# wenzhang-dev/bitcaskDB

Measured on AMD Instinct MI355X. Metric: WAL record decode+CRC GiB/s (device-resident), 4 KiB values, 1/2/4/8 MI355X, higher is better.
Workload: dtype u8; 1 GPU; config B: 1073743514 B WAL segment per GPU, NsSize 20, 100 B keys, 4 KiB values, device-resident decode+CRC+record parse; seg_bytes=1073743514, records=253846, fragments=286402, parallelism=one independent segment per GPU x1

## Files before the change

### bitcaskdb_amd/csrc/bcw_api.cpp

```cpp
#include <hip/hip_runtime.h>
#include <nmmintrin.h>

#include <algorithm>
#include <atomic>
#include <cmath>
#include <cstdlib>
#include <cstring>
#include <new>
#include <thread>
#include <vector>

#include "bcw.h"
#include "bcw_internal.h"

namespace bcw {

static void byte_table(uint32_t* t0) {
  for (uint32_t b = 0; b < 256; ++b) {
    uint32_t c = b;
    for (int k = 0; k < 8; ++k) c = (c >> 1) ^ (0x82F63B78u & (0u - (c & 1u)));
    t0[b] = c;
  }
}

static inline uint32_t zero_step(const uint32_t* t0, uint32_t s) { return (s >> 8) ^ t0[s & 0xffu]; }

static void shift_basis(const uint32_t* t0, uint64_t n, uint32_t* img) {
  for (int i = 0; i < 32; ++i) {
    uint32_t v = 1u << i;
    for (uint64_t k = 0; k < n; ++k) v = zero_step(t0, v);
    img[i] = v;
  }
}
static inline uint32_t apply_basis(const uint32_t* img, uint32_t x) {
  uint32_t r = 0;
  for (int i = 0; x; ++i, x >>= 1)
    if (x & 1u) r ^= img[i];
  return r;
}

static void invert_basis(const uint32_t* img, uint32_t* inv) {
  uint32_t out[32], in[32];
  for (int i = 0; i < 32; ++i) { out[i] = img[i]; in[i] = 1u << i; }
  for (int bit = 0; bit < 32; ++bit) {
    int p = bit;
    while (p < 32 && !((out[p] >> bit) & 1u)) ++p;
    std::swap(out[bit], out[p]);
    std::swap(in[bit], in[p]);
    for (int r = 0; r < 32; ++r)
      if (r != bit && ((out[r] >> bit) & 1u)) { out[r] ^= out[bit]; in[r] ^= in[bit]; }
  }
  for (int bit = 0; bit < 32; ++bit) inv[bit] = in[bit];
}

static void nibble_image(const uint32_t* img, uint32_t* t) {
  for (int i = 0; i < 8; ++i)
    for (uint32_t n = 0; n < 16; ++n) t[i * 16 + n] = apply_basis(img, n << (4 * i));
}

static void build_enc_ops(uint32_t* ops) {
  uint32_t t0[256];
  byte_table(t0);
  uint32_t img[32], inv[32], sq[32];
  for (int n = 0; n < 16; ++n) { shift_basis(t0, 16ull * n, img); nibble_image(img, ops + n * 128); }
  for (int n = 0; n < 16; ++n) { shift_basis(t0, 256ull * n, img); nibble_image(img, ops + (16 + n) * 128); }
  for (int n = 0; n < 8; ++n) { shift_basis(t0, 4096ull * n, img); nibble_image(img, ops + (32 + n) * 128); }
  for (int t = 0; t < 16; ++t) {
    shift_basis(t0, (uint64_t)t, img);
    invert_basis(img, inv);
    nibble_image(inv, ops + (kOpInv + t) * 128);
  }
  shift_basis(t0, 1, img);
  for (int k = 0; k < 32; ++k) {
    nibble_image(img, ops + (kOpPow2 + k) * 128);
    if (k < 15) {
      invert_basis(img, inv);
      nibble_image(inv, ops + (kOpPow2Inv + k) * 128);
    }
    for (int i = 0; i < 32; ++i) sq[i] = apply_basis(img, img[i]);
    memcpy(img, sq, sizeof img);
  }
}

void build_initc(uint32_t* initc) {
  uint32_t t0[256];
  byte_table(t0);
  uint32_t v = 0xffffffffu;
  for (uint32_t L = 0; L <= kBlock; ++L) {
    initc[L] = v;
    v = zero_step(t0, v);
  }
}

static uint32_t crc32c_hw(const uint8_t* p, size_t n) {
  uint64_t c = 0xffffffffu;
  while (n >= 8) {
    uint64_t w;
    memcpy(&w, p, 8);
    c = _mm_crc32_u64(c, w);
    p += 8;
    n -= 8;
  }
  uint32_t c32 = (uint32_t)c;
  while (n--) c32 = _mm_crc32_u8(c32, *p++);
  return ~c32;
}
static inline uint32_t mask_crc(uint32_t c) { return ((c >> 15) | (c << 17)) + 0xa282ead8u; }

}

using namespace bcw;


#define HIPCHK(x)                          \
  do {                                     \
    if ((x) != hipSuccess) return BCW_E_HIP; \
  } while (0)

namespace {
std::atomic<uint64_t> g_ctx_ids{1};
}

extern "C" {

int bcw_abi_version(void) { return BCW_ABI_VERSION; }

const char* bcw_strerror(int code) {
  switch (code) {
    case BCW_OK: return "ok";
    case BCW_E_INVAL: return "invalid argument";
    case BCW_E_HIP: return "HIP runtime error";
    case BCW_E_NOMEM: return "out of memory";
    case BCW_E_CAPACITY: return "output capacity too small";
    case BCW_E_NODEVICE: return "no HIP device";
    case BCW_E_IO: return "file read / write failed";
    default: return "unknown error";
  }
}

int bcw_device_count(void) {
  int n = 0;
  if (hipGetDeviceCount(&n) != hipSuccess) return 0;
  return n;
}

uint32_t bcw_crc32c_masked(const uint8_t* p, uint64_t n) { return mask_crc(crc32c_hw(p, (size_t)n)); }

void bcw_write_super_block(uint8_t out[40], uint64_t create_time, uint64_t base_time) {
  memset(out, 0, 40);
  const uint64_t magic = BCW_MAGIC, bs = BCW_BLOCK_SIZE;
  const uint32_t so = BCW_SUPER_BLOCK_SIZE;
  memcpy(out + 0, &magic, 8);
  memcpy(out + 8, &bs, 8);
  memcpy(out + 16, &so, 4);
  memcpy(out + 20, &create_time, 8);
  memcpy(out + 28, &base_time, 8);
  const uint32_t crc = bcw_crc32c_masked(out, 36);
  memcpy(out + 36, &crc, 4);
}

int bcw_load_super_block(const uint8_t* p, uint64_t n, bcw_super_block* out) {
  if (!p || !out) return BCW_E_INVAL;
  if (n < BCW_SUPER_BLOCK_SIZE) return BCW_SB_SHORT;
  uint32_t want;
  memcpy(&want, p + 36, 4);
  const uint32_t crc = bcw_crc32c_masked(p, 36);
  if (crc != want) return BCW_SB_CRC;
  memcpy(&out->magic, p, 8);
  if (out->magic != BCW_MAGIC) return BCW_SB_MAGIC;
  memcpy(&out->block_size, p + 8, 8);
  memcpy(&out->start_off, p + 16, 4);
  if (out->block_size != BCW_BLOCK_SIZE) return BCW_SB_BLOCKSIZE;
  memcpy(&out->create_time, p + 20, 8);
  memcpy(&out->base_time, p + 28, 8);
  out->crc = crc;
  return BCW_SB_OK;
}

uint64_t bcw_wal_record_size(uint64_t offset, uint64_t size) {
  uint64_t left = size, phy = 0;
  offset -= BCW_SUPER_BLOCK_SIZE;
  while (left > 0) {
    uint64_t leftover = BCW_BLOCK_SIZE - (offset % BCW_BLOCK_SIZE);
    if (leftover < BCW_HEADER_SIZE) {
      phy += leftover;
      offset += leftover;
      leftover = BCW_BLOCK_SIZE;
    }
    const uint64_t frag = std::min(left, leftover - BCW_HEADER_SIZE);
    phy += BCW_HEADER_SIZE + frag;
    offset += BCW_HEADER_SIZE + frag;
    left -= frag;
  }
  return phy;
}

void bcw_wal_block_index_range(uint64_t offset, uint64_t size, uint64_t* first_blk_idx, uint64_t* first_blk_off,
                               uint64_t* blk_num) {
  const uint64_t rs = bcw_wal_record_size(offset, size);
  const uint64_t first = (offset - BCW_SUPER_BLOCK_SIZE) / BCW_BLOCK_SIZE;
  const uint64_t last = (offset - BCW_SUPER_BLOCK_SIZE + rs) / BCW_BLOCK_SIZE;
  if (first_blk_idx) *first_blk_idx = first;
  if (first_blk_off) *first_blk_off = first * BCW_BLOCK_SIZE + BCW_SUPER_BLOCK_SIZE;
  if (blk_num) *blk_num = last - first + 1;
}

uint64_t bcw_max_fragments(uint64_t seg_len, uint32_t start_off) {
  if (seg_len <= start_off) return 0;
  return (seg_len - start_off) / BCW_HEADER_SIZE + 1;
}

int bcw_ctx_create(int device, bcw_ctx** out) {
  if (!out) return BCW_E_INVAL;
  *out = nullptr;
  int n = 0;
  if (hipGetDeviceCount(&n) != hipSuccess || n == 0) return BCW_E_NODEVICE;
  if (device < 0 || device >= n) return BCW_E_INVAL;
  bcw_ctx* c = new (std::nothrow) bcw_ctx();
  if (!c) return BCW_E_NOMEM;
  c->device = device;
  c->id = g_ctx_ids.fetch_add(1);
  DeviceGuard dg(device);
  if (!dg.ok) { delete c; return BCW_E_HIP; }
  hipDeviceProp_t prop;
  if (hipGetDeviceProperties(&prop, device) == hipSuccess && prop.multiProcessorCount > 0)
    c->num_cus = prop.multiProcessorCount;
  if (hipStreamCreateWithFlags(&c->own, hipStreamNonBlocking) != hipSuccess) { delete c; return BCW_E_HIP; }
  c->cur = c->own;
  std::vector<uint32_t> initc(kBlock + 1);
  build_initc(initc.data());
  std::vector<uint32_t> enc_ops(kEncOpsWords);
  build_enc_ops(enc_ops.data());
  std::vector<uint32_t> pow2(kPow2Ops * 128);
  {
    uint32_t t0[256], img[32], sq[32];
    byte_table(t0);
    shift_basis(t0, 1, img);
    for (int k = 0; k < kPow2Ops; ++k) {
      nibble_image(img, pow2.data() + k * 128);
      for (int i = 0; i < 32; ++i) sq[i] = apply_basis(img, img[i]);
      memcpy(img, sq, sizeof img);
    }
  }
  std::vector<uint32_t> image2(kS2Image);
  {
    uint32_t tk[4][256], t0[256], img[32], nib[128], step[32], m[32];
    byte_table(t0);
    memcpy(tk[0], t0, sizeof t0);
    for (int k = 1; k < 4; ++k)
      for (int e = 0; e < 256; ++e) tk[k][e] = (tk[k - 1][e] >> 8) ^ t0[tk[k - 1][e] & 0xffu];
    uint32_t sh[32];
    shift_basis(t0, kSChunk - kSPiece, sh);
    for (int e = 0; e < 256; ++e)
      for (int s = 0; s < 4; ++s)
        for (int cp = 0; cp < 8; ++cp) {
          image2[kS2SliceOff + e * 64 + s * 8 + cp] = tk[3 - s][e];
          image2[kS2SliceOff + e * 64 + 32 + s * 8 + cp] = apply_basis(sh, tk[3 - s][e]);
        }
    shift_basis(t0, kSPiece, step);
    for (int i = 0; i < 32; ++i) m[i] = 1u << i;
    for (int l = 63; l >= 0; --l) {
      nibble_image(m, nib);
      for (int k = 0; k < 128; ++k) image2[kS2LopOff + k * 64 + l] = nib[k];
      for (int i = 0; i < 32; ++i) m[i] = apply_basis(step, m[i]);
    }
    for (int k = 0; k < kSPW; ++k) {
      shift_basis(t0, 4u * (kSPW - k) + (kSChunk - kSPiece), img);
      for (int t = 0; t < 4; ++t)
        for (uint32_t e = 0; e < 256; ++e)
          image2[kS2KopOff + (k * 4 + t) * 256 + e] = apply_basis(img, e << (8 * t));
    }
    auto put_bytes = [&](int at, const uint8_t (&b)[16]) {
      for (int w = 0; w < 4; ++w)
        image2[at + w] = b[4 * w] | b[4 * w + 1] << 8 | b[4 * w + 2] << 16 | (uint32_t)b[4 * w + 3] << 24;
    };
    for (int n = 0; n < kS2GeN; ++n) {
      uint8_t b[16];
      for (int q = 0; q < 16; ++q) b[q] = q >= n ? 0xff : 0x00;
      put_bytes(kS2Ge + 4 * n, b);
    }
    for (int m = 0; m < kS2JselN; ++m) {
      uint8_t b[16];
      for (int q = 0; q < 16; ++q) {
        const int p = q - (m - 3);
        b[q] = (m < kS2JselN - 1 && p >= 0 && p < 4) ? (uint8_t)(4 + p) : 0x0c;
      }
      put_bytes(kS2Jsel + 4 * m, b);
    }
    for (int g = 0; g < kS2GapN; ++g) {
      uint8_t b[16];
      for (int q = 0; q < 16; ++q) {
        const int p = q - (g - 6);
        b[q] = g == kS2GapN - 1 ? (uint8_t)(q & 3) : (p >= 0 && p < 4) ? (uint8_t)(4 + p) : (p >= 4 && p < 7) ? 0x0c
                                                                                            : (uint8_t)(q & 3);
      }
      put_bytes(kS2Gap + 4 * g, b);
    }
  }
  bool ok = hipMalloc(&c->tabs.lds_image2, image2.size() * 4) == hipSuccess &&
            hipMemcpy(c->tabs.lds_image2, image2.data(), image2.size() * 4, hipMemcpyHostToDevice) == hipSuccess;
  ok = ok && hipMalloc(&c->tabs.initc, initc.size() * 4) == hipSuccess &&
            hipMalloc(&c->tabs.enc_ops, enc_ops.size() * 4) == hipSuccess &&
            hipMalloc(&c->tabs.pow2, pow2.size() * 4) == hipSuccess &&
            hipMalloc(&c->d_eres, sizeof(bcw_encode_result)) == hipSuccess &&
            hipMalloc(&c->d_result, sizeof(bcw_decode_result)) == hipSuccess &&
            hipMalloc(&c->d_ires, sizeof(bcw_index_result)) == hipSuccess;
  ok = ok && hipMemcpy(c->tabs.initc, initc.data(), initc.size() * 4, hipMemcpyHostToDevice) == hipSuccess &&
       hipMemcpy(c->tabs.enc_ops, enc_ops.data(), enc_ops.size() * 4, hipMemcpyHostToDevice) == hipSuccess &&
       hipMemcpy(c->tabs.pow2, pow2.data(), pow2.size() * 4, hipMemcpyHostToDevice) == hipSuccess;
  if (!ok) { bcw_ctx_destroy(c); return BCW_E_NOMEM; }
  *out = c;
  return BCW_OK;
}

static void free_scratch(Scratch& s) {
  (void)hipFree(s.fbase);
  (void)hipFree(s.rbase);
  (void)hipFree(s.bsum);
  (void)hipFree(s.lb);
  (void)hipFree(s.lbe);
  (void)hipFree(s.frags);
  (void)hipFree(s.srec);
  (void)hipFree(s.fok);
  (void)hipFree(s.wstart);
  (void)hipFree(s.xbal);
  (void)hipFree(s.misc);
  s = Scratch{};
}

static void free_enc_scratch(EncScratch& e) {
  void* ptrs[] = {e.sz,    e.mflag, e.dsrc, e.da,      e.hda,       e.hsz,  e.dpos,
                  e.hpos,  e.tiles, e.ev,   e.evb,     e.recdesc,   e.emisc, e.evt,
                  e.hnl,   e.evw,   e.wl};
  for (void* q : ptrs) (void)hipFree(q);
  hipStream_t aux = e.aux;
  hipEvent_t evs[3] = {e.ev_scan, e.ev_hscan, e.ev_desc};
  e = EncScratch{};
  e.aux = aux;
  e.ev_scan = evs[0];
  e.ev_hscan = evs[1];
  e.ev_desc = evs[2];
}

int bcw_ctx_destroy(bcw_ctx* c) {
  if (!c) return BCW_E_INVAL;
  DeviceGuard dg(c->device);
  if (c->cur) (void)hipStreamSynchronize(c->cur);
  free_scratch(c->s);
  free_enc_scratch(c->es);
  if (c->es.aux) (void)hipStreamSynchronize(c->es.aux);
  if (c->es.ev_scan) (void)hipEventDestroy(c->es.ev_scan);
  if (c->es.ev_hscan) (void)hipEventDestroy(c->es.ev_hscan);
  if (c->es.ev_desc) (void)hipEventDestroy(c->es.ev_desc);
  if (c->es.aux) (void)hipStreamDestroy(c->es.aux);
  (void)hipFree(c->tabs.enc_ops);
  (void)hipFree(c->tabs.pow2);
  (void)hipFree(c->d_keep);
  (void)hipFree(c->d_eout);
  (void)hipFree(c->d_eres);
  (void)hipFree(c->tabs.initc);
  (void)hipFree(c->tabs.lds_image2);
  (void)hipFree(c->d_seg);
  (void)hipFree(c->d_tab_mem);
  (void)hipFree(c->d_result);
  (void)hipFree(c->d_ires);
  for (auto& m : c->prof.marks) { (void)hipEventDestroy(m.a); (void)hipEventDestroy(m.b); }
  for (auto e : c->prof.pool) (void)hipEventDestroy(e);
  if (c->own) (void)hipStreamDestroy(c->own);
  delete c;
  return BCW_OK;
}

int bcw_ctx_set_stream(bcw_ctx* c, void* stream) {
  if (!c) return BCW_E_INVAL;
  c->cur = stream ? (hipStream_t)stream : c->own;
  return BCW_OK;
}
void* bcw_ctx_stream(bcw_ctx* c) { return c ? (void*)c->cur : nullptr; }
int bcw_ctx_device(bcw_ctx* c) { return c ? c->device : -1; }
int bcw_ctx_sync(bcw_ctx* c) {
  if (!c) return BCW_E_INVAL;
  return hipStreamSynchronize(c->cur) == hipSuccess ? BCW_OK : BCW_E_HIP;
}

static int ensure_scratch(bcw_ctx* c, uint64_t nblocks, uint64_t frag_cap) {
  Scratch& s = c->s;
  if (nblocks <= s.nblocks_cap && frag_cap <= s.frag_cap && s.misc) return BCW_OK;
  (void)hipStreamSynchronize(c->cur);
  const uint64_t nb = std::max(nblocks, s.nblocks_cap);
  const uint64_t fc = std::max(frag_cap, s.frag_cap);
  free_scratch(s);
  const uint64_t nwg = std::max<uint64_t>(nb / 64 + 2, (uint64_t)c->num_cus + 2);
  bool ok = hipMalloc(&s.fbase, (nb + 1) * 4) == hipSuccess && hipMalloc(&s.rbase, (nb + 1) * 4) == hipSuccess &&
            hipMalloc(&s.bsum, (nb + 1) * sizeof(uint2)) == hipSuccess && hipMalloc(&s.lb, nwg * 8) == hipSuccess &&
            hipMalloc(&s.lbe, nwg * 8) == hipSuccess && hipMalloc(&s.frags, fc * sizeof(Frag)) == hipSuccess &&
            hipMalloc(&s.srec, (fc + 4) * sizeof(uint4)) == hipSuccess &&
            hipMalloc(&s.fok, fc) == hipSuccess &&
            hipMalloc(&s.wstart, ((size_t)c->num_cus * kCrcWaves + 1) * 4) == hipSuccess &&
            hipMalloc(&s.xbal, sizeof(XBal)) == hipSuccess &&
            hipMalloc(&s.misc, 16 * sizeof(uint64_t)) == hipSuccess;
  if (!ok) { free_scratch(s); return BCW_E_NOMEM; }
  s.nblocks_cap = nb;
  s.frag_cap = fc;
  s.nlb = nwg;
  s.epoch = 1;
  s.chase_direct = c->chase_direct;
  XBal xb{};
  for (uint32_t y = 0; y < 8; ++y) xb.w[y] = 65536u;
  if (hipMemcpyHtoDAsync(s.xbal, &xb, sizeof xb, c->cur) != hipSuccess || hipStreamSynchronize(c->cur) != hipSuccess ||
      hipMemsetAsync(s.lb, 0, nwg * 8, c->cur) != hipSuccess || hipMemsetAsync(s.lbe, 0, nwg * 8, c->cur) != hipSuccess ||
      hipMemsetAsync(s.misc, 0, 16 * sizeof(uint64_t), c->cur) != hipSuccess ||
      hipMemsetAsync(s.misc + 14, 0xff, 2 * sizeof(uint64_t), c->cur) != hipSuccess ||
      hipMemsetAsync(s.misc, 0xff, sizeof(uint64_t), c->cur) != hipSuccess) {
    free_scratch(s);
    return BCW_E_HIP;
  }
  return BCW_OK;
}

int bcw_decode_segment_async(bcw_ctx* c, const uint8_t* d_seg, const bcw_decode_params* p,
                             const bcw_record_table* t, bcw_decode_result* d_result) {
  if (!c || !p || !t || !d_result) return BCW_E_INVAL;
  if (p->mode != BCW_MODE_RECORD && p->mode != BCW_MODE_HINT) return BCW_E_INVAL;
  if (!t->foff || !t->size || !t->expire || !t->key_len || !t->val_len || !t->meta_len || !t->first_frag ||
      !t->emit_frag || !t->hdr_size || !t->flags || !t->etag_off || !t->status)
    return BCW_E_INVAL;
  if (p->mode == BCW_MODE_HINT && (!t->aux0 || !t->aux1)) return BCW_E_INVAL;
  if (p->seg_len > BCW_MAX_SEGMENT) return BCW_E_INVAL;
  DeviceGuard dg(c->device);
  if (!dg.ok) return BCW_E_HIP;
  c->last_start_off = p->start_off;
  const uint64_t gen = (c->id << 32) | (++c->gen_seq & 0xffffffffull);
  c->frag_gen = gen;
  bcw_decode_result r{};
  r.err_frag = ~0ull;
  r.first_bad_record = -1;
  r.generation = gen;
  if ((uint64_t)p->start_off > p->seg_len) {
    r.err_class = BCW_ERR_PANIC;
    HIPCHK(hipMemcpyAsync(d_result, &r, sizeof r, hipMemcpyHostToDevice, c->cur));
    return BCW_OK;
  }
  const uint64_t nblocks = (p->seg_len - p->start_off + kBlock - 1) / kBlock;
  if (nblocks == 0 || !d_seg) {
    if (nblocks != 0) return BCW_E_INVAL;
    HIPCHK(hipMemcpyAsync(d_result, &r, sizeof r, hipMemcpyHostToDevice, c->cur));
    return BCW_OK;
  }
  const uint64_t per = p->mode == BCW_MODE_HINT ? 96 : 256;
  uint64_t want = std::max<uint64_t>(65536, (p->seg_len - p->start_off) / per + nblocks * 2);
  want = std::max(want, c->frag_hint);
  want = std::min(want, bcw_max_fragments(p->seg_len, p->start_off) + 64);
  want = std::min<uint64_t>(want, 0xfffffff0ull);
  int rc = ensure_scratch(c, nblocks, want);
  if (rc != BCW_OK) return rc;
  c->s.test_abort_wg = c->test_abort_wg;
  c->test_abort_wg = 0;
  if (launch_decode(d_seg, *p, *t, d_result, c->tabs, c->s, nblocks, gen, c->cur, c->num_cus, &c->prof) !=
      hipSuccess)
    return BCW_E_HIP;
  return BCW_OK;
}

int bcw_decode_fragments_async(bcw_ctx* c, const bcw_frag_table* d_frags) {
  if (!c || !d_frags) return BCW_E_INVAL;
  if (!c->s.misc) return BCW_OK;
  DeviceGuard dg(c->device);
  if (!dg.ok) return BCW_E_HIP;
  const uint64_t n = std::min(c->s.frag_cap, d_frags->capacity);
  return launch_export_frags(c->s, *d_frags, c->last_start_off, c->cur, n, c->tabs.initc) == hipSuccess ? BCW_OK
                                                                                                  : BCW_E_HIP;
}

static const char* kKernelNames[K_NUM] = {"k_chase", "k_crc", "(retired)", "k_enc_prep", "k_enc_scan", "k_events",
                                          "k_write", "k_hint_layout", "k_events_hint"};

int bcw_ctx_reserve_fragments(bcw_ctx* c, uint64_t n) {
  if (!c || n >= 0xfffffff0ull) return BCW_E_INVAL;
  c->frag_hint = std::max(c->frag_hint, n);
  return BCW_OK;
}

int bcw_ctx_set_option(bcw_ctx* c, int option, uint64_t value) {
  if (!c) return BCW_E_INVAL;
  switch (option) {
    case BCW_OPT_CHASE_DIRECT:
      if (value > BCW_CHASE_DIRECT_MAX) return BCW_E_INVAL;
      c->s.chase_direct = (uint32_t)value;
      c->chase_direct = (uint32_t)value;
      return BCW_OK;
    case BCW_OPT_DECODE_PATH:
    case BCW_OPT_DECODE_CHUNKS:
      return value == 1 ? BCW_OK : BCW_E_INVAL;
    case BCW_OPT_XCD_BALANCE:
      if (value > 1) return BCW_E_INVAL;
      c->s.xbal_on = (uint32_t)value;
      return BCW_OK;
    case BCW_OPT_FILTER_SNAPSHOT:
      if (value > 1) return BCW_E_INVAL;
      c->filter_snapshot = value != 0;
      return BCW_OK;
    case BCW_OPT_TEST_ABORT_WAIT: {
      const char* hooks = getenv("BCW_TEST_HOOKS");
      if (!hooks || strcmp(hooks, "1") != 0 || value > 0xffffffffull) return BCW_E_INVAL;
      c->test_abort_wg = value;
      return BCW_OK;
    }
    default:
      return BCW_E_INVAL;
  }
}

int bcw_ctx_set_profiling(bcw_ctx* c, int mask) {
  if (!c) return BCW_E_INVAL;
  c->prof.mask = (uint32_t)mask;
  return BCW_OK;
}

int bcw_ctx_set_profiling_sample(bcw_ctx* c, int every) {
  if (!c || every < 1) return BCW_E_INVAL;
  c->prof.every = (uint32_t)every;
  for (uint32_t& q : c->prof.seq) q = 0;
  return BCW_OK;
}

int bcw_ctx_kernel_times(bcw_ctx* c, double* total_ms, uint64_t* launches, int n) {
  if (!c || n < 0) return BCW_E_INVAL;
  if (hipStreamSynchronize(c->cur) != hipSuccess) return BCW_E_HIP;
  for (int k = 0; k < n; ++k) { if (total_ms) total_ms[k] = 0; if (launches) launches[k] = 0; }
  for (const auto& m : c->prof.marks) {
    float ms = 0;
    if (m.kid < n && hipEventElapsedTime(&ms, m.a, m.b) == hipSuccess) {
      if (total_ms) total_ms[m.kid] += ms;
      if (launches) launches[m.kid] += 1;
    }
    c->prof.pool.push_back(m.a);
    c->prof.pool.push_back(m.b);
  }
  c->prof.marks.clear();
  return K_NUM;
}

const char* bcw_kernel_name(int kid) { return (kid >= 0 && kid < K_NUM) ? kKernelNames[kid] : nullptr; }

int bcw_decode_fragments(bcw_ctx* c, const bcw_frag_table* h, uint64_t* n_total) {
  if (!c || !h) return BCW_E_INVAL;
  if (n_total) *n_total = 0;
  if (!c->s.misc) return BCW_OK;
  DeviceGuard dg(c->device);
  if (!dg.ok) return BCW_E_HIP;
  uint64_t misc[16];
  HIPCHK(hipMemcpyAsync(misc, c->s.misc, sizeof misc, hipMemcpyDeviceToHost, c->cur));
  HIPCHK(hipStreamSynchronize(c->cur));
  const uint64_t total = std::min(misc[4], c->s.frag_cap);
  if (n_total) *n_total = total;
  const uint64_t n = std::min(total, h->capacity);
  if (n == 0) return BCW_OK;
  void* mem = nullptr;
  if (hipMalloc(&mem, n * 19) != hipSuccess) return BCW_E_NOMEM;
  uint8_t* m = (uint8_t*)mem;
  bcw_frag_table d;
  d.capacity = n;
  d.data_off = (uint64_t*)m; m += n * 8;
  d.len = (uint32_t*)m; m += n * 4;
  d.stored_crc = (uint32_t*)m; m += n * 4;
  d.type = m; m += n;
  d.crc_ok = m;
  bool ok = launch_export_frags(c->s, d, c->last_start_off, c->cur, n, c->tabs.initc) == hipSuccess;
  auto cp = [&](void* dst, const void* src, size_t esz) {
    return !dst || hipMemcpyAsync(dst, src, n * esz, hipMemcpyDeviceToHost, c->cur) == hipSuccess;
  };
  ok = ok && cp(h->data_off, d.data_off, 8) && cp(h->len, d.len, 4) && cp(h->stored_crc, d.stored_crc, 4) &&
       cp(h->type, d.type, 1) && cp(h->crc_ok, d.crc_ok, 1);
  ok = ok && hipStreamSynchronize(c->cur) == hipSuccess;
  (void)hipFree(mem);
  return ok ? BCW_OK : BCW_E_HIP;
}

static int ensure_dev_table(bcw_ctx* c, uint64_t cap, bool hint) {
  if (cap <= c->d_tab_cap && c->d_tab_mem) return BCW_OK;
  (void)hipStreamSynchronize(c->cur);
  (void)hipFree(c->d_tab_mem);
  c->d_tab_mem = nullptr;
  const uint64_t n = std::max<uint64_t>(cap, 1);
  const size_t bytes = n * (8 * 5 + 4 * 5 + 4);
  if (hipMalloc(&c->d_tab_mem, bytes) != hipSuccess) { c->d_tab_cap = 0; return BCW_E_NOMEM; }
  uint8_t* m = (uint8_t*)c->d_tab_mem;
  bcw_record_table& t = c->d_tab;
  t.capacity = n;
  t.foff = (uint64_t*)m; m += n * 8;
  t.size = (uint64_t*)m; m += n * 8;
  t.expire = (uint64_t*)m; m += n * 8;
  t.aux0 = (uint64_t*)m; m += n * 8;
  t.aux1 = (uint64_t*)m; m += n * 8;
  t.key_len = (uint32_t*)m; m += n * 4;
  t.val_len = (uint32_t*)m; m += n * 4;
  t.meta_len = (uint32_t*)m; m += n * 4;
  t.first_frag = (uint32_t*)m; m += n * 4;
  t.emit_frag = (uint32_t*)m; m += n * 4;
  t.hdr_size = m; m += n;
  t.flags = m; m += n;
  t.etag_off = m; m += n;
  t.status = m;
  c->d_tab_cap = n;
  (void)hint;
  return BCW_OK;
}

int bcw_decode_segment(bcw_ctx* c, const uint8_t* h_seg, const bcw_decode_params* p,
                       const bcw_record_table* h, bcw_decode_result* h_result) {
  if (!c || !p || !h || !h_result) return BCW_E_INVAL;
  if (p->seg_len && !h_seg) return BCW_E_INVAL;
  DeviceGuard dg(c->device);
  if (!dg.ok) return BCW_E_HIP;
  if (p->seg_len > c->d_seg_cap) {
    (void)hipStreamSynchronize(c->cur);
    (void)hipFree(c->d_seg);
    c->d_seg = nullptr;
    c->d_seg_cap = 0;
    if (hipMalloc(&c->d_seg, p->seg_len) != hipSuccess) return BCW_E_NOMEM;
    c->d_seg_cap = p->seg_len;
  }
  if (p->seg_len) HIPCHK(hipMemcpyAsync(c->d_seg, h_seg, p->seg_len, hipMemcpyHostToDevice, c->cur));
  int rc = ensure_dev_table(c, h->capacity, p->mode == BCW_MODE_HINT);
  if (rc != BCW_OK) return rc;
  for (int attempt = 0; attempt < 3; ++attempt) {
    rc = bcw_decode_segment_async(c, c->d_seg, p, &c->d_tab, c->d_result);
    if (rc != BCW_OK) return rc;
    HIPCHK(hipMemcpyAsync(h_result, c->d_result, sizeof *h_result, hipMemcpyDeviceToHost, c->cur));
    HIPCHK(hipStreamSynchronize(c->cur));
    if (!h_result->retry_frag_capacity) break;
    if (bcw_ctx_reserve_fragments(c, h_result->retry_frag_capacity + 64) != BCW_OK) return BCW_E_CAPACITY;
  }
  if (h_result->retry_frag_capacity) return BCW_E_NOMEM;
  const uint64_t n = std::min(h_result->n_records, h->capacity);
  const bcw_record_table& d = c->d_tab;
  auto cp = [&](void* dst, const void* src, size_t esz) -> bool {
    if (!dst || n == 0) return true;
    return hipMemcpyAsync(dst, src, n * esz, hipMemcpyDeviceToHost, c->cur) == hipSuccess;
  };
  bool ok = cp(h->foff, d.foff, 8) && cp(h->size, d.size, 8) && cp(h->expire, d.expire, 8) &&
            cp(h->aux0, d.aux0, 8) && cp(h->aux1, d.aux1, 8) && cp(h->key_len, d.key_len, 4) &&
            cp(h->val_len, d.val_len, 4) && cp(h->meta_len, d.meta_len, 4) && cp(h->first_frag, d.first_frag, 4) &&
            cp(h->emit_frag, d.emit_frag, 4) && cp(h->hdr_size, d.hdr_size, 1) && cp(h->flags, d.flags, 1) &&
            cp(h->etag_off, d.etag_off, 1) && cp(h->status, d.status, 1);
  if (!ok) return BCW_E_HIP;
  HIPCHK(hipStreamSynchronize(c->cur));
  return h_result->n_records > h->capacity ? BCW_E_CAPACITY : BCW_OK;
}


static int ensure_enc_scratch(bcw_ctx* c, uint64_t rows) {
  EncScratch& e = c->es;
  if (rows <= e.rows_cap && e.emisc) return BCW_OK;
  (void)hipStreamSynchronize(c->cur);
  const uint64_t r = std::max(std::max(rows, e.rows_cap), (uint64_t)1);
  free_enc_scratch(e);
  const uint64_t ntiles = r / enc_tile_items() + 2;
  const uint64_t nwin = r / enc_ev_win() + 2;
  bool ok = hipMalloc(&e.sz, r * 4) == hipSuccess && hipMalloc(&e.mflag, r) == hipSuccess &&
            hipMalloc(&e.dsrc, r * 4) == hipSuccess && hipMalloc(&e.da, (r + 1) * 8) == hipSuccess &&
            hipMalloc(&e.hda, (r + 1) * 8) == hipSuccess && hipMalloc(&e.hsz, r * 4) == hipSuccess &&
            hipMalloc(&e.dpos, r * 8) == hipSuccess && hipMalloc(&e.hpos, r * 8) == hipSuccess &&
            hipMalloc(&e.tiles, ntiles * enc_sizeof_tile()) == hipSuccess &&
            hipMalloc(&e.ev, (r + 2) * enc_sizeof_ev()) == hipSuccess && hipMalloc(&e.evb, nwin * 4) == hipSuccess &&
            hipMalloc(&e.evt, nwin * 32768 * 8) == hipSuccess && hipMalloc(&e.hnl, r * 2) == hipSuccess &&
            hipMalloc(&e.evw, nwin * 12) == hipSuccess &&
            hipMalloc(&e.recdesc, r * enc_sizeof_recdesc()) == hipSuccess && hipMalloc(&e.wl, r * 4) == hipSuccess &&
            hipMalloc(&e.emisc, 64 * sizeof(uint64_t)) == hipSuccess;
  if (!ok) { free_enc_scratch(e); return BCW_E_NOMEM; }
  if (!e.aux && (hipStreamCreateWithFlags(&e.aux, hipStreamNonBlocking) != hipSuccess ||
                 hipEventCreateWithFlags(&e.ev_scan, hipEventDisableTiming) != hipSuccess ||
                 hipEventCreateWithFlags(&e.ev_hscan, hipEventDisableTiming) != hipSuccess ||
                 hipEventCreateWithFlags(&e.ev_desc, hipEventDisableTiming) != hipSuccess))
    return BCW_E_HIP;
  (void)hipMemsetAsync(e.mflag, 0, r, c->cur);
  e.rows_cap = r;
  return BCW_OK;
}

int bcw_encode_segment_async(bcw_ctx* c, const uint8_t* d_src, const bcw_encode_params* p,
                             const bcw_record_table* t, const bcw_decode_result* d_src_result, const uint8_t* d_keep,
                             const bcw_encode_out* o, bcw_encode_result* d_result) {
  if (!c || !p || !t || !d_src_result || !o || !d_result) return BCW_E_INVAL;
  if (p->mode != BCW_ENC_COMPACT && p->mode != BCW_ENC_HINT) return BCW_E_INVAL;
  if (p->hint_pos < BCW_SUPER_BLOCK_SIZE || !o->hint) return BCW_E_INVAL;
  if (p->mode == BCW_ENC_COMPACT && (p->wal_pos < BCW_SUPER_BLOCK_SIZE || !o->wal || !d_keep)) return BCW_E_INVAL;
  if (!t->foff || !t->size || !t->expire || !t->key_len || !t->val_len || !t->meta_len || !t->first_frag ||
      !t->emit_frag || !t->hdr_size || !t->flags || !t->etag_off || !t->status)
    return BCW_E_INVAL;
  if (!c->s.frags) return BCW_E_INVAL;
  if (t->capacity >= 0xffffff00ull) return BCW_E_INVAL;
  DeviceGuard dg(c->device);
  if (!dg.ok) return BCW_E_HIP;
  int rc = ensure_enc_scratch(c, t->capacity);
  if (rc != BCW_OK) return rc;
  EncLaunch L{};
  L.d_src = d_src;
  L.p = *p;
  L.table = *t;
  L.rows = t->capacity;
  L.d_src_result = d_src_result;
  L.d_keep = d_keep;
  L.out = *o;
  L.d_result = d_result;
  L.frags = c->s.frags;
  L.crc_ops = c->tabs.enc_ops;
  L.initc = c->tabs.initc;
  L.num_cus = c->num_cus;
  L.gen = c->frag_gen;
  return launch_encode(L, c->es, c->cur, &c->prof) == hipSuccess ? BCW_OK : BCW_E_HIP;
}

}

namespace bcw {
int sync_decode(bcw_ctx* c, const uint8_t* h_src, const bcw_decode_params& dp, bcw_decode_result& dres) {
  uint64_t cap = std::max<uint64_t>(16, dp.seg_len / 64 + 16);
  if (dp.seg_len > c->d_seg_cap) {
    (void)hipStreamSynchronize(c->cur);
    (void)hipFree(c->d_seg);
    c->d_seg = nullptr;
    c->d_seg_cap = 0;
    if (hipMalloc(&c->d_seg, dp.seg_len) != hipSuccess) return BCW_E_NOMEM;
    c->d_seg_cap = dp.seg_len;
  }
  if (dp.seg_len) HIPCHK(hipMemcpyAsync(c->d_seg, h_src, dp.seg_len, hipMemcpyHostToDevice, c->cur));
  for (;;) {
    int rc = ensure_dev_table(c, cap, dp.mode == BCW_MODE_HINT);
    if (rc != BCW_OK) return rc;
    for (int attempt = 0; attempt < 3; ++attempt) {
      rc = bcw_decode_segment_async(c, c->d_seg, &dp, &c->d_tab, c->d_result);
      if (rc != BCW_OK) return rc;
      HIPCHK(hipMemcpyAsync(&dres, c->d_result, sizeof dres, hipMemcpyDeviceToHost, c->cur));
      HIPCHK(hipStreamSynchronize(c->cur));
      if (!dres.retry_frag_capacity) break;
      if (bcw_ctx_reserve_fragments(c, dres.retry_frag_capacity + 64) != BCW_OK) return BCW_E_CAPACITY;
    }
    if (dres.retry_frag_capacity) return BCW_E_NOMEM;
    if (dres.n_records <= c->d_tab.capacity) return BCW_OK;
    cap = dres.n_records + 16;
  }
}

int ensure_keep(bcw_ctx* c, uint64_t rows) {
  if (rows <= c->d_keep_cap && c->d_keep) return BCW_OK;
  (void)hipStreamSynchronize(c->cur);
  (void)hipFree(c->d_keep);
  c->d_keep = nullptr;
  c->d_keep_cap = 0;
  if (hipMalloc(&c->d_keep, std::max<uint64_t>(rows, 1)) != hipSuccess) return BCW_E_NOMEM;
  c->d_keep_cap = std::max<uint64_t>(rows, 1);
  return BCW_OK;
}

bcw_decode_params src_params(const uint8_t* h_src, const bcw_encode_params* p) {
  bcw_super_block sb{};
  bcw_decode_params dp{};
  dp.seg_len = p->src_len;
  dp.start_off = p->src_start_off;
  dp.ns_size = p->ns_size;
  dp.etag_size = p->etag_size;
  dp.mode = BCW_MODE_RECORD;
  dp.base_time = (bcw_load_super_block(h_src, p->src_len, &sb) == BCW_SB_OK) ? sb.base_time : 0;
  return dp;
}

int encode_run(bcw_ctx* c, const bcw_encode_params* p, const bcw_encode_out* h, bcw_encode_result* h_result,
               bcw_encode_out* d_out) {
  const uint64_t rows = c->d_tab.capacity;
  const uint64_t need = h->wal_cap + h->hint_cap + rows * 8;
  if (need > c->d_eout_cap) {
    (void)hipStreamSynchronize(c->cur);
    (void)hipFree(c->d_eout);
    c->d_eout = nullptr;
    c->d_eout_cap = 0;
    if (hipMalloc(&c->d_eout, need + 64) != hipSuccess) return BCW_E_NOMEM;
    c->d_eout_cap = need;
  }
  uint8_t* m = (uint8_t*)c->d_eout;
  bcw_encode_out& d = *d_out;
  d = bcw_encode_out{};
  d.rec_off = (uint64_t*)m;
  d.rec_off_cap = rows;
  m += rows * 8;
  d.wal = m;
  d.wal_cap = h->wal_cap;
  m += (h->wal_cap + 15) & ~15ull;
  d.hint = (uint8_t*)(((uintptr_t)m + 15) & ~(uintptr_t)15);
  d.hint_cap = h->hint_cap;
  if (p->mode == BCW_ENC_HINT && !d.wal) d.wal = d.hint;
  int rc = bcw_encode_segment_async(c, c->d_seg, p, &c->d_tab, c->d_result, c->d_keep, &d, c->d_eres);
  if (rc != BCW_OK) return rc;
  HIPCHK(hipMemcpyAsync(h_result, c->d_eres, sizeof *h_result, hipMemcpyDeviceToHost, c->cur));
  HIPCHK(hipStreamSynchronize(c->cur));
  if (!h_result->fits) return BCW_E_CAPACITY;
  if (h->rec_off && h->rec_off_cap < h_result->n_in) return BCW_E_CAPACITY;
  return BCW_OK;
}

int encode_copy_out(bcw_ctx* c, const bcw_encode_params* p, const bcw_encode_out* h, const bcw_encode_result& r,
                    const bcw_encode_out& d, const bcw_decode_result& dres) {
  if (h->wal && r.wal_need && p->mode == BCW_ENC_COMPACT)
    HIPCHK(hipMemcpyAsync(h->wal, d.wal, r.wal_need, hipMemcpyDeviceToHost, c->cur));
  if (h->hint && r.hint_need) HIPCHK(hipMemcpyAsync(h->hint, d.hint, r.hint_need, hipMemcpyDeviceToHost, c->cur));
  const uint64_t nr = std::min(r.n_in, d.rec_off_cap);
  if (h->rec_off && nr) HIPCHK(hipMemcpyAsync(h->rec_off, d.rec_off, nr * 8, hipMemcpyDeviceToHost, c->cur));
  HIPCHK(hipStreamSynchronize(c->cur));
  if (h->rec_off)
    for (uint64_t i = nr; i < h->rec_off_cap && i < dres.n_records; ++i) h->rec_off[i] = ~0ull;
  return BCW_OK;
}

int encode_to_host(bcw_ctx* c, const bcw_encode_params* p, const bcw_encode_out* h, bcw_encode_result* h_result,
                   const bcw_decode_result& dres) {
  bcw_encode_out d{};
  const int rc = encode_run(c, p, h, h_result, &d);
  return rc != BCW_OK ? rc : encode_copy_out(c, p, h, *h_result, d, dres);
}
}

extern "C" {

int bcw_encode_segment(bcw_ctx* c, const uint8_t* h_src, const bcw_encode_params* p, const uint8_t* h_keep,
                       uint64_t n_keep, const bcw_encode_out* h, bcw_encode_result* h_result) {
  if (!c || !p || !h || !h_result) return BCW_E_INVAL;
  if (p->src_len && !h_src) return BCW_E_INVAL;
  DeviceGuard dg(c->device);
  if (!dg.ok) return BCW_E_HIP;
  const bcw_decode_params dp = src_params(h_src, p);
  bcw_decode_result dres{};
  int rc = sync_decode(c, h_src, dp, dres);
  if (rc != BCW_OK) return rc;
  const uint64_t rows = c->d_tab.capacity;
  rc = ensure_keep(c, rows);
  if (rc != BCW_OK) return rc;
  HIPCHK(hipMemsetAsync(c->d_keep, 0, rows, c->cur));
  const uint64_t nk = std::min(n_keep, rows);
  if (h_keep && nk) HIPCHK(hipMemcpyAsync(c->d_keep, h_keep, nk, hipMemcpyHostToDevice, c->cur));
  return encode_to_host(c, p, h, h_result, dres);
}

int bcw_compact_segment(bcw_ctx* c, bcw_index* ix, const uint8_t* h_src, const bcw_encode_params* p, uint64_t src_fid,
                        const bcw_encode_out* h, bcw_encode_result* h_result, bcw_index_result* h_filter) {
  if (!c || !ix || !p || !h || !h_result || p->mode != BCW_ENC_COMPACT) return BCW_E_INVAL;
  if (index_ctx(ix) != c) return BCW_E_INVAL;
  if (p->src_len && !h_src) return BCW_E_INVAL;
  DeviceGuard dg(c->device);
  if (!dg.ok) return BCW_E_HIP;
  const bcw_decode_params dp = src_params(h_src, p);
  bcw_decode_result dres{};
  int rc = sync_decode(c, h_src, dp, dres);
  if (rc != BCW_OK) return rc;
  rc = ensure_keep(c, c->d_tab.capacity);
  if (rc != BCW_OK) return rc;
  rc = bcw_compact_filter_async(ix, c->d_seg, &dp, &c->d_tab, c->d_result, src_fid, c->d_keep,
                                h_filter ? c->d_ires : nullptr);
  if (rc != BCW_OK) return rc;
  if (h_filter) HIPCHK(hipMemcpyAsync(h_filter, c->d_ires, sizeof *h_filter, hipMemcpyDeviceToHost, c->cur));
  return encode_to_host(c, p, h, h_result, dres);
}

int bcw_index_recover_segment(bcw_ctx* c, bcw_index* ix, const uint8_t* h_seg, const bcw_decode_params* p,
                              uint64_t fid, int use_record_fid, bcw_decode_result* h_dres,
                              bcw_index_result* h_out) {
  if (!c || !ix || !p || !h_out) return BCW_E_INVAL;
  if (index_ctx(ix) != c) return BCW_E_INVAL;
  if (p->seg_len && !h_seg) return BCW_E_INVAL;
  DeviceGuard dg(c->device);
  if (!dg.ok) return BCW_E_HIP;
  bcw_decode_result dres{};
  int rc = sync_decode(c, h_seg, *p, dres);
  if (rc != BCW_OK) return rc;
  if (h_dres) *h_dres = dres;
  rc = bcw_index_put_decoded_async(ix, c->d_seg, p, &c->d_tab, c->d_result, fid, use_record_fid, c->d_ires);
  if (rc != BCW_OK) return rc;
  HIPCHK(hipMemcpyAsync(h_out, c->d_ires, sizeof *h_out, hipMemcpyDeviceToHost, c->cur));
  HIPCHK(hipStreamSynchronize(c->cur));
  return BCW_OK;
}

namespace {
struct Writer {
  uint8_t* out;
  uint64_t cap;
  uint64_t len;
  void put(const void* p, uint64_t n) {
    if (out && len + n <= cap) memcpy(out + len, p, n);
    len += n;
  }
  uint64_t write_record(const uint8_t* rec, uint64_t n, bool compute_crc) {
    static const uint8_t pad[6] = {0, 0, 0, 0, 0, 0};
    uint64_t offset = 0, left = n;
    bool begin = true;
    while (left > 0) {
      uint64_t leftover = BCW_BLOCK_SIZE - ((len - BCW_SUPER_BLOCK_SIZE) % BCW_BLOCK_SIZE);
      if (leftover < BCW_HEADER_SIZE) {
        put(pad, leftover);
        leftover = BCW_BLOCK_SIZE;
      }
      if (begin) offset = len;
      const uint64_t avail = leftover - BCW_HEADER_SIZE;
      const uint64_t frag = std::min(left, avail);
      const bool end = left == frag;
      const uint8_t type = (begin && end) ? BCW_RECORD_FULL : begin ? BCW_RECORD_FIRST : end ? BCW_RECORD_LAST
                                                                                          : BCW_RECORD_MIDDLE;
      uint8_t hdr[7];
      const uint32_t crc = compute_crc ? mask_crc(crc32c_hw(rec, frag)) : 0;
      const uint16_t l16 = (uint16_t)frag;
      memcpy(hdr, &crc, 4);
      memcpy(hdr + 4, &l16, 2);
      hdr[6] = type;
      put(hdr, 7);
      put(rec, frag);
      rec += frag;
      left -= frag;
      begin = false;
    }
    return offset;
  }
};

inline uint64_t splitmix64(uint64_t& s) {
  uint64_t z = (s += 0x9E3779B97F4A7C15ull);
  z = (z ^ (z >> 30)) * 0xBF58476D1CE4E5B9ull;
  z = (z ^ (z >> 27)) * 0x94D049BB133111EBull;
  return z ^ (z >> 31);
}
inline void fill_rand(uint64_t& s, uint8_t* p, size_t n) {
  size_t i = 0;
  for (; i + 8 <= n; i += 8) {
    const uint64_t v = splitmix64(s);
    memcpy(p + i, &v, 8);
  }
  if (i < n) {
    const uint64_t v = splitmix64(s);
    memcpy(p + i, &v, n - i);
  }
}
inline int put_uvarint(uint8_t* o, uint64_t v) {
  int i = 0;
  while (v >= 0x80) { o[i++] = (uint8_t)(v | 0x80); v >>= 7; }
  o[i++] = (uint8_t)v;
  return i;
}
}

int bcw_synth_segment(uint64_t target_bytes, uint64_t max_records, uint64_t seed, uint32_t ns_size,
                      uint32_t key_len, uint32_t value_len, int value_mode, uint64_t base_time, uint8_t* h_out,
                      uint64_t out_cap, uint64_t* out_len, uint64_t* out_records) {
  if (value_mode != 0 && value_mode != 1) return BCW_E_INVAL;
  if (ns_size > 255 || key_len > (1u << 20) || value_len > (1u << 26)) return BCW_E_INVAL;
  Writer w0{h_out, out_cap, 0};
  uint8_t sb[40];
  bcw_write_super_block(sb, base_time, base_time);
  w0.put(sb, 40);
  std::vector<double> cdf;
  if (value_mode == 1) {
    cdf.resize(512);
    double acc = 0;
    for (int k = 1; k <= 512; ++k) { acc += std::pow((double)k, -1.1); cdf[k - 1] = acc; }
    for (auto& x : cdf) x /= acc;
  }
  const size_t vmax = value_mode == 1 ? 128 * 512 : value_len;
  std::vector<uint8_t> ns(ns_size);
  for (uint32_t i = 0; i < ns_size; ++i) ns[i] = (uint8_t)('A' + i % 26);
  struct Bufs {
    std::vector<uint8_t> key, val, rec;
  };
  auto one = [&](uint64_t i, uint64_t& s, Writer& w, bool fill, Bufs& B) {
    size_t vl = value_len;
    if (value_mode == 1) {
      const double u = (double)(splitmix64(s) >> 11) * (1.0 / 9007199254740992.0);
      vl = 128u * (size_t)(std::lower_bound(cdf.begin(), cdf.end(), u) - cdf.begin() + 1);
    }
    if (fill) {
      fill_rand(s, B.key.data(), key_len);
      if (key_len >= 8) memcpy(B.key.data(), &i, 8);
      fill_rand(s, B.val.data(), vl);
    } else {
      s += 0x9E3779B97F4A7C15ull * (uint64_t)(((key_len + 7) / 8) + ((vl + 7) / 8));
    }
    uint8_t tmp[30];
    int t = 0;
    t += put_uvarint(tmp + t, key_len);
    t += put_uvarint(tmp + t, vl);
    t += put_uvarint(tmp + t, 0);
    const size_t header = (size_t)t + ns_size + 2;
    const size_t n = header + key_len + vl;
    if (!fill) {
      w.write_record(B.rec.data(), n, false);
      return;
    }
    uint8_t* r = B.rec.data();
    size_t o = 0;
    r[o++] = (uint8_t)header;
    memcpy(r + o, ns.data(), ns_size); o += ns_size;
    r[o++] = (uint8_t)((1u << 0) | (1u << 1));
    memcpy(r + o, tmp, t); o += t;
    memcpy(r + o, B.key.data(), key_len); o += key_len;
    memcpy(r + o, B.val.data(), vl); o += vl;
    w.write_record(r, o, true);
  };
  auto bufs = [&]() {
    Bufs B;
    B.key.resize(key_len + 8);
    B.val.resize(vmax + 8);
    B.rec.resize(vmax + key_len + ns_size + 64);
    return B;
  };
  constexpr uint64_t kCk = 4096;
  struct Ck {
    uint64_t i, s, len;
  };
  std::vector<Ck> ck;
  Writer wl{nullptr, 0, w0.len};
  uint64_t s = seed, n = 0;
  Bufs B0 = bufs();
  for (uint64_t i = 0; (max_records == 0 || i < max_records) && wl.len < target_bytes; ++i) {
    if (i % kCk == 0) ck.push_back(Ck{i, s, wl.len});
    one(i, s, wl, false, B0);
    ++n;
  }
  if (out_len) *out_len = wl.len;
  if (out_records) *out_records = n;
  if (!h_out) return BCW_OK;
  if (wl.len > out_cap) return BCW_E_CAPACITY;
  const unsigned hw = std::thread::hardware_concurrency();
  const uint64_t nth = std::max<uint64_t>(1, std::min<uint64_t>({(uint64_t)(hw ? hw : 1), 16, ck.size()}));
  std::atomic<uint64_t> next{0};
  auto fill = [&]() {
    Bufs B = bufs();
    for (uint64_t c; (c = next.fetch_add(1)) < ck.size();) {
      Writer w{h_out, out_cap, ck[c].len};
      uint64_t st = ck[c].s;
      const uint64_t i1 = std::min<uint64_t>(ck[c].i + kCk, n);
      for (uint64_t i = ck[c].i; i < i1; ++i) one(i, st, w, true, B);
    }
  };
  std::vector<std::thread> pool;
  for (uint64_t t = 1; t < nth; ++t) pool.emplace_back(fill);
  fill();
  for (auto& t : pool) t.join();
  return BCW_OK;
}

}
```

### bitcaskdb_amd/csrc/bcw_decode.hip

```cpp
#include <hip/hip_runtime.h>

#include <cstdint>

#include "bcw_internal.h"
#include "bcw_parse.h"

namespace bcw {

enum { M_FIRST_BAD = 0,
       M_NE = 1,
       M_NFRAGS = 4, M_DONE_CRC = 5,
       M_T_CRC0 = 10, M_T_FIN = 11,
       M_ABORT = 12,
       M_BAD_CRC = 14,
       M_BAD_TYPE = 15 };

__device__ __forceinline__ uint32_t rotl32(uint32_t x, int r) { return (x << r) | (x >> (32 - r)); }

__device__ __forceinline__ void read_header(const uint8_t* __restrict__ seg, uint64_t seg_len, uint64_t off,
                                            uint32_t& crc, uint32_t& len, uint32_t& type) {
  const uint64_t a = off & ~3ull;
  uint32_t w0, w1, w2;
  if (a + 12 <= seg_len) {
    const uint32_t* q = reinterpret_cast<const uint32_t*>(seg + a);
    w0 = q[0]; w1 = q[1]; w2 = q[2];
  } else {
    uint32_t b[12];
#pragma unroll
    for (int i = 0; i < 12; ++i) b[i] = (a + i < seg_len) ? seg[a + i] : 0u;
    w0 = b[0] | b[1] << 8 | b[2] << 16 | b[3] << 24;
    w1 = b[4] | b[5] << 8 | b[6] << 16 | b[7] << 24;
    w2 = b[8] | b[9] << 8 | b[10] << 16 | b[11] << 24;
  }
  const uint32_t sh = (uint32_t)(off & 3);
  crc = __builtin_amdgcn_alignbyte(w1, w0, sh);
  const uint32_t t = __builtin_amdgcn_alignbyte(w2, w1, sh);
  len = t & 0xffffu;
  type = (t >> 16) & 0xffu;
}

__device__ __forceinline__ uint32_t wave_incl_scan_u32(uint32_t v, uint32_t lane) {
#pragma unroll
  for (int d = 1; d < 64; d <<= 1) {
    const uint32_t t = __shfl_up(v, d, 64);
    if (lane >= (uint32_t)d) v += t;
  }
  return v;
}
template <int CTRL>
__device__ __forceinline__ uint32_t dpp_mov(uint32_t v) {
  return (uint32_t)__builtin_amdgcn_mov_dpp((int)v, CTRL, 0xf, 0xf, false);
}
template <int CTRL, int ROWMASK = 0xf>
__device__ __forceinline__ uint32_t dpp_z(uint32_t v) {
  return (uint32_t)__builtin_amdgcn_update_dpp(0, (int)v, CTRL, ROWMASK, 0xf, true);
}
template <typename Op>
__device__ __forceinline__ uint32_t wave_scan_z(uint32_t v, Op op) {
  v = op(v, dpp_z<0x111>(v));
  v = op(v, dpp_z<0x112>(v));
  v = op(v, dpp_z<0x114>(v));
  v = op(v, dpp_z<0x118>(v));
  v = op(v, dpp_z<0x142, 0xa>(v));
  v = op(v, dpp_z<0x143, 0xc>(v));
  return v;
}
__device__ __forceinline__ uint32_t wave_max_scan(uint32_t v, uint32_t) {
  return wave_scan_z(v, [](uint32_t x, uint32_t y) { return max(x, y); });
}
__device__ __forceinline__ uint32_t wave_or_scan(uint32_t v, uint32_t) {
  return wave_scan_z(v, [](uint32_t x, uint32_t y) { return x | y; });
}
__device__ __forceinline__ uint32_t wave_add_scan(uint32_t v, uint32_t) {
  return wave_scan_z(v, [](uint32_t x, uint32_t y) { return x + y; });
}

__device__ __forceinline__ uint32_t wg256_excl_scan(uint32_t v, uint32_t* sm4, uint32_t& total) {
  const uint32_t lane = threadIdx.x & 63u, wave = threadIdx.x >> 6;
  const uint32_t incl = wave_incl_scan_u32(v, lane);
  if (lane == 63) sm4[wave] = incl;
  __syncthreads();
  uint32_t base = 0;
  for (uint32_t k = 0; k < wave; ++k) base += sm4[k];
  total = sm4[0] + sm4[1] + sm4[2] + sm4[3];
  __syncthreads();
  return base + incl - v;
}

struct Spin {
  uint64_t t0 = 0;
  uint64_t lim = 20000000ull;
  __device__ __forceinline__ bool go(uint64_t* misc, uint32_t site) {
    const uint64_t t = wall_clock64();
    if (t0 == 0) t0 = t;
    if (t - t0 < lim &&
        __hip_atomic_load(&misc[M_ABORT], __ATOMIC_RELAXED, __HIP_MEMORY_SCOPE_AGENT) == 0ull) {
      __builtin_amdgcn_s_sleep(1);
      return true;
    }
    atomicMax(reinterpret_cast<unsigned long long*>(&misc[M_ABORT]), (unsigned long long)site);
    return false;
  }
};

constexpr int kChaseHold = 64;
constexpr uint64_t kLbAgg = 1, kLbInc = 2, kLbMask = (1ull << 38) - 1;
constexpr int kDirect = BCW_CHASE_DIRECT_MAX;

template <typename V>
__device__ __forceinline__ uint32_t chase_block(const uint8_t* __restrict__ seg, uint64_t seg_len, uint64_t boff,
                                                uint32_t bufsize, V&& visit, uint32_t h = 0, uint32_t n = 0) {
  while (h + kHdr <= bufsize) {
    uint32_t crc, len, type;
    read_header(seg, seg_len, boff + h, crc, len, type);
    const uint32_t start = h + kHdr;
    if (len > bufsize - start) len = bufsize - start;
    visit(n, start, len, crc, type);
    ++n;
    h = start + len;
  }
  return n;
}

constexpr uint32_t kRecUsual = 1u << 20, kRecAdj = 1u << 21;
__device__ __forceinline__ uint32_t check_word(uint32_t crc, uint32_t ic) { return ~rotl32(crc - 0xa282ead8u, 15) ^ ic; }
__device__ __forceinline__ void put_frag_J(Frag* __restrict__ frags, uint4* __restrict__ srec, uint64_t g,
                                           uint64_t frag_cap, uint32_t b, uint64_t boff, uint32_t start_len,
                                           uint32_t J, uint32_t type, bool adj) {
  if (g >= frag_cap) return;
  *reinterpret_cast<uint4*>(frags + g) = make_uint4(b, start_len, J, type & 0xffu);
  const uint64_t gs = boff + (start_len & 0xffffu), ge = gs + (start_len >> 16);
  const uint32_t cb = (uint32_t)(gs / kSChunk), ce = (uint32_t)(ge / kSChunk);
  const uint32_t pa = (uint32_t)(gs % kSChunk), pb = (uint32_t)(ge % kSChunk);
  const bool usual = adj && cb < ce && pb <= (uint32_t)kSChunk - 8u;
  const uint32_t e = pb + 4u, K = ((e % kSPiece) + 3u) >> 2, Lfull = e / kSPiece + (K == (uint32_t)kSPW ? 1u : 0u);
  srec[g] = make_uint4(ce, cb, J, pb | pa << 10 | (usual ? kRecUsual : 0u) | (adj ? kRecAdj : 0u) | Lfull << 22 |
                                      (K & 3u) << 29);
}
__device__ __forceinline__ void put_frag(Frag* __restrict__ frags, uint4* __restrict__ srec, uint64_t g,
                                         uint64_t frag_cap, uint32_t b, uint64_t boff, uint32_t start, uint32_t len,
                                         uint32_t crc, uint32_t type, const uint32_t* __restrict__ initc, bool adj) {
  put_frag_J(frags, srec, g, frag_cap, b, boff, start | (len << 16), check_word(crc, initc[len]), type, adj);
}

constexpr uint32_t kSumHasE = 1u << 16;

struct ClassW {
  uint64_t pw;
  uint64_t pp0, pp1;
  uint64_t p8;
  __device__ __forceinline__ uint64_t weight(uint32_t y) const {
    return (uint64_t)(65536 + 256 * (int64_t)(int8_t)(uint8_t)(pw >> (8u * y)));
  }
  __device__ __forceinline__ uint64_t prefix(uint32_t y) const {
    const uint64_t f = (y < 4u ? pp0 : pp1) >> (16u * (y & 3u));
    return (uint64_t)(65536 * (int64_t)y + 256 * (int64_t)(int16_t)(uint16_t)f);
  }
  __device__ __forceinline__ uint32_t classes_below(double x) const {
    uint32_t n = 0;
#pragma unroll
    for (uint32_t k = 1; k < 8; ++k) n += (double)prefix(k) <= x ? 1u : 0u;
    return n;
  }
};
__device__ __forceinline__ uint64_t div_floor(uint64_t a, uint64_t b, double rb) {
  uint64_t q = (uint64_t)((double)a * rb);
  while (q * b > a) --q;
  while ((q + 1) * b <= a) ++q;
  return q;
}
struct WavePart {
  ClassW cw;
  uint64_t L, nwaves, round16, den16, C;
  double rden, rC;
  __device__ __forceinline__ WavePart(const ClassW& c, uint64_t L_, uint64_t nwaves_) : cw(c), L(L_), nwaves(nwaves_) {
    const uint32_t G = (uint32_t)(nwaves / kCrcWaves);
    round16 = 16ull * cw.p8;
    den16 = round16 * (G / 8u) + 16ull * cw.prefix(G % 8u);
    C = L / 1024u;
    rden = 1.0 / (double)den16;
    rC = C ? 1.0 / (double)C : 0.0;
  }
  __device__ __forceinline__ uint64_t P(uint64_t v) const {
    if (v >= nwaves) return L;
    const uint64_t r = v / kCrcWaves;
    const uint32_t y = (uint32_t)(r % 8u);
    const uint64_t num16 = round16 * (r / 8u) + 16ull * cw.prefix(y) + cw.weight(y) * (v % kCrcWaves);
    return 1024u * div_floor(num16 * C, den16, rden);
  }
  __device__ __forceinline__ uint64_t first_at(uint64_t x) const {
    if (C == 0) return x == 0 ? 0 : nwaves;
    const uint64_t X = (x + 1023u) / 1024u, N = div_floor(X * den16 + C - 1, C, rC);
    const uint32_t q = (uint32_t)N / (uint32_t)round16;
    const uint64_t rem = N - (uint64_t)q * round16;
    uint32_t y = 0;
#pragma unroll
    for (uint32_t k = 1; k < 8; ++k) y += 16ull * cw.prefix(k) <= rem ? 1u : 0u;
    const uint64_t wy = cw.weight(y), base = 16ull * cw.prefix(y);
    const uint32_t jj = (uint32_t)(rem - base + wy - 1) / (uint32_t)wy;
    const uint64_t v = ((uint64_t)q * 8u + y) * kCrcWaves + jj;
    return v < nwaves ? v : nwaves;
  }
};

__device__ __forceinline__ ClassW class_weights(uint32_t xw) {
  ClassW c{0, 0, 0, 0};
  int64_t acc = 0;
#pragma unroll
  for (int k = 0; k < 8; ++k) {
    const int64_t d = ((int64_t)__builtin_amdgcn_readlane(xw, k) - 65536) / 256;
    c.pw |= (uint64_t)(uint8_t)(int8_t)d << (8 * k);
    if (k < 4) c.pp0 |= (uint64_t)(uint16_t)(int16_t)acc << (16 * k);
    else c.pp1 |= (uint64_t)(uint16_t)(int16_t)acc << (16 * (k - 4));
    acc += d;
  }
  c.p8 = (uint64_t)(65536 * 8 + 256 * acc);
  return c;
}

template <int ABL = 0>
__global__ __launch_bounds__(64) void k_chase(const uint8_t* __restrict__ seg, uint64_t seg_len, uint32_t start_off,
                                              uint64_t nblocks, uint32_t* __restrict__ fbase,
                                              uint32_t* __restrict__ rbase, uint2* __restrict__ bsum,
                                              Frag* __restrict__ frags, uint4* __restrict__ srec, uint64_t frag_cap,
                                              uint64_t* __restrict__ lb,
                                              uint64_t* __restrict__ lbe, uint64_t* __restrict__ misc,
                                              uint64_t epoch, const uint32_t* __restrict__ initc,
                                              uint32_t direct_max, uint64_t test_abort_wg,
                                              uint32_t* __restrict__ wstart, uint32_t nwaves,
                                              XBal* __restrict__ xb, uint32_t xb_on) {
  constexpr int kHold = (ABL & 256) ? 16 : kChaseHold;
  __shared__ uint32_t s_hold[kHold][2][64];
  __shared__ uint8_t s_type[kHold][64];
  const uint32_t lane = threadIdx.x;
  const uint32_t xw = lane < 8u ? (xb_on ? xb->w[lane] : 65536u) : 0u;
  const uint64_t tc0 = (ABL & 16) ? __builtin_amdgcn_s_memtime() : 0;
  if ((ABL & 32) && threadIdx.x == 0) lbe[4 * blockIdx.x] = wall_clock64();
  const uint64_t wg = blockIdx.x;
  if (wg >= (nblocks + 63) / 64) return;
  const uint64_t b = wg * 64 + lane;
  uint32_t bufsize = 0;
  uint64_t boff = 0;
  if (b < nblocks) {
    boff = (uint64_t)start_off + b * kBlock;
    bufsize = (uint32_t)((seg_len - boff) < kBlock ? (seg_len - boff) : kBlock);
  }
  uint32_t ne = 0, tacc = 0, tnz = 0xffffu, tst = 0, badk = 0xffffffffu;
  uint32_t hres = 0;
  const uint32_t n = chase_block(seg, seg_len, boff, bufsize,
                                 [&](uint32_t k, uint32_t start, uint32_t len, uint32_t crc, uint32_t type) {
                                   if (k < (uint32_t)kHold) {
                                     s_hold[k][0][lane] = crc;
                                     s_hold[k][1][lane] = start | (len << 16);
                                     s_type[k][lane] = (uint8_t)type;
                                   }
                                   if (k == (uint32_t)kHold - 1u) hres = start + len;
                                   if (type == BCW_RECORD_FULL || type == BCW_RECORD_LAST) {
                                     ++ne;
                                     tacc = 0;
                                     tnz = 0xffffu;
                                   } else {
                                     if (len > 0 && tnz == 0xffffu) { tnz = k; tst = start; }
                                     tacc += len;
                                     if ((type < BCW_RECORD_FULL || type > BCW_RECORD_LAST) && badk == 0xffffffffu) badk = k;
                                   }
                                 });
  const uint64_t tc1 = (ABL & 16) ? __builtin_amdgcn_s_memtime() : 0;
  if ((ABL & 32) && lane == 0) lbe[4 * wg + 1] = wall_clock64();
  if (wg == 0 && lane == 0) xb->on = xb_on;
  const uint32_t incl = wave_add_scan(n, lane);
  const uint32_t tot = __builtin_amdgcn_readlane(incl, 63);
  const uint32_t incl_e = wave_add_scan(ne, lane);
  const uint32_t tot_e = __builtin_amdgcn_readlane(incl_e, 63);
  const uint64_t tag = epoch << 40;
  const uint64_t nwg_all = (nblocks + 63) / 64;
  const bool force = wg + 1 == test_abort_wg;
  uint64_t excl = 0, excl_e = 0;
  const uint32_t nh = n < (uint32_t)kHold ? n : (uint32_t)kHold;
  auto held_checks = [&]() {
    if (ABL & 2) return;
    constexpr uint32_t kWb = 16;
    static_assert(kHold % kWb == 0, "held-header batches stay inside s_hold");
    for (uint32_t k0 = 0; k0 < nh; k0 += kWb) {
      uint32_t ic[kWb];
#pragma unroll
      for (uint32_t q = 0; q < kWb; ++q) ic[q] = initc[k0 + q < nh ? s_hold[k0 + q][1][lane] >> 16 : 0u];
#pragma unroll
      for (uint32_t q = 0; q < kWb; ++q)
        if (k0 + q < nh) s_hold[k0 + q][0][lane] = check_word(s_hold[k0 + q][0][lane], ic[q]);
    }
  };
  if (ABL & 1) {
    held_checks();
  } else if (nwg_all <= (uint64_t)direct_max) {
    if (lane == 0)
      __hip_atomic_store(&lb[wg], tag | (kLbAgg << 38) | tot | ((uint64_t)tot_e << 19), __ATOMIC_RELAXED,
                         __HIP_MEMORY_SCOPE_AGENT);
    uint64_t v[kDirect / 64];
#pragma unroll
    for (int k = 0; k < kDirect / 64; ++k) {
      const uint64_t q = lane + 64u * k;
      v[k] = q < wg ? __hip_atomic_load(&lb[q], __ATOMIC_RELAXED, __HIP_MEMORY_SCOPE_AGENT) : tag;
    }
    held_checks();
    Spin sp;
    if (force) sp.lim = 0;
    for (;;) {
      bool wait = force;
#pragma unroll
      for (int k = 0; k < kDirect / 64; ++k) wait |= (v[k] >> 40) != epoch;
      if (!__builtin_amdgcn_readfirstlane((uint32_t)(__ballot(wait) != 0ull))) break;
      if (!sp.go(misc, 9)) {
#pragma unroll
        for (int k = 0; k < kDirect / 64; ++k)
          if ((v[k] >> 40) != epoch) v[k] = 0;
        break;
      }
#pragma unroll
      for (int k = 0; k < kDirect / 64; ++k) {
        const uint64_t q = lane + 64u * k;
        if ((v[k] >> 40) != epoch) v[k] = __hip_atomic_load(&lb[q], __ATOMIC_RELAXED, __HIP_MEMORY_SCOPE_AGENT);
      }
    }
    uint64_t c = 0, ce = 0;
#pragma unroll
    for (int k = 0; k < kDirect / 64; ++k) {
      const uint64_t q = lane + 64u * k;
      if (q < wg) {
        c += v[k] & 0x7ffffu;
        ce += (v[k] >> 19) & 0x7ffffu;
      }
    }
#pragma unroll
    for (int d = 32; d >= 1; d >>= 1) {
      c += (uint64_t)__shfl_xor((long long)c, d, 64);
      ce += (uint64_t)__shfl_xor((long long)ce, d, 64);
    }
    excl = c;
    excl_e = ce;
  } else {
    const uint64_t fl = (wg == 0 ? kLbInc : kLbAgg) << 38;
    if (lane == 0) {
      __hip_atomic_store(&lb[wg], tag | fl | tot, __ATOMIC_RELAXED, __HIP_MEMORY_SCOPE_AGENT);
      __hip_atomic_store(&lbe[wg], tag | fl | tot_e, __ATOMIC_RELAXED, __HIP_MEMORY_SCOPE_AGENT);
    }
    held_checks();
    bool dn = false, de = false;
    for (uint64_t top = wg; top > 0 && !(dn && de);) {
      const uint64_t q = top - 1 - lane;
      uint64_t vn = 0, ve = 0;
      if (top > lane) {
        Spin sp;
        if (force) sp.lim = 0;
        if (!dn)
          while (((vn = __hip_atomic_load(&lb[q], __ATOMIC_RELAXED, __HIP_MEMORY_SCOPE_AGENT)) >> 40) != epoch || force)
            if (!sp.go(misc, 10)) { vn = 0; break; }
        if (!de)
          while (((ve = __hip_atomic_load(&lbe[q], __ATOMIC_RELAXED, __HIP_MEMORY_SCOPE_AGENT)) >> 40) != epoch || force)
            if (!sp.go(misc, 11)) { ve = 0; break; }
      }
      auto step = [&](uint64_t v, bool& done, uint64_t& acc) {
        if (done) return;
        const uint64_t inc = __ballot(top > lane && ((v >> 38) & 3u) == kLbInc);
        const uint32_t stop = inc ? (uint32_t)__builtin_ctzll(inc) : 64u;
        uint64_t c = (lane <= stop && top > lane) ? (v & kLbMask) : 0ull;
#pragma unroll
        for (int d = 32; d >= 1; d >>= 1) c += (uint64_t)__shfl_xor((long long)c, d, 64);
        acc += c;
        done = inc != 0;
      };
      step(vn, dn, excl);
      step(ve, de, excl_e);
      top = top > 64 ? top - 64 : 0;
    }
    if (lane == 0 && wg != 0) {
      __hip_atomic_store(&lb[wg], tag | (kLbInc << 38) | ((excl + tot) & kLbMask), __ATOMIC_RELAXED,
                         __HIP_MEMORY_SCOPE_AGENT);
      __hip_atomic_store(&lbe[wg], tag | (kLbInc << 38) | ((excl_e + tot_e) & kLbMask), __ATOMIC_RELAXED,
                         __HIP_MEMORY_SCOPE_AGENT);
    }
  }
  const uint64_t g0 = excl + incl - n;
  const uint64_t tc2 = (ABL & 16) ? __builtin_amdgcn_s_memtime() : 0;
  if ((ABL & 32) && lane == 0) lbe[4 * wg + 2] = wall_clock64();
  if (b < nblocks && !(ABL & 2)) {
    fbase[b] = (uint32_t)(g0 < 0xffffffffull ? g0 : 0xffffffffull);
    const uint64_t r0 = excl_e + incl_e - ne;
    rbase[b] = (uint32_t)(r0 < 0xffffffffull ? r0 : 0xffffffffull);
    bsum[b] = make_uint2(tacc | (tnz << 16), tst | (ne ? kSumHasE : 0u));
    if (badk != 0xffffffffu)
      atomicMin(reinterpret_cast<unsigned long long*>(&misc[M_BAD_TYPE]), (unsigned long long)(g0 + badk));
    const bool next_hdr = b + 1 < nblocks && seg_len - (boff + kBlock) >= kHdr;
    auto adj = [&](uint32_t k, uint32_t sl_k) { return k + 1u < n || (next_hdr && (sl_k & 0xffffu) + (sl_k >> 16) == kBlock); };
    const uint64_t L = seg_len - start_off, rel = boff - start_off;
    const WavePart wp(class_weights(xw), L, nwaves);
    const uint64_t span = b + 1 == nblocks ? ~0ull : (uint64_t)kBlock - 1;
    uint64_t w = wp.first_at(rel);
    uint64_t bw = wp.P(w) - rel;
    auto bounds_upto = [&](uint64_t hp, uint64_t idx) __attribute__((always_inline)) {
      const uint64_t h = hp < span ? hp : span;
      while (w <= nwaves && bw <= h) {
        wstart[w] = (uint32_t)(idx < 0xffffffffull ? idx : 0xffffffffull);
        ++w;
        bw = wp.P(w) - rel;
      }
    };
    for (uint32_t k = 0; k < nh; ++k) {
      const uint32_t sl = s_hold[k][1][lane];
      put_frag_J(frags, srec, g0 + k, frag_cap, (uint32_t)b, boff, sl, s_hold[k][0][lane], s_type[k][lane],
                 adj(k, sl));
      bounds_upto((sl & 0xffffu) - kHdr, g0 + k);
    }
    if (n > (uint32_t)kHold)
      chase_block(seg, seg_len, boff, bufsize, [&](uint32_t k, uint32_t start, uint32_t len, uint32_t crc, uint32_t type) {
        put_frag(frags, srec, g0 + k, frag_cap, (uint32_t)b, boff, start, len, crc, type, initc,
                 adj(k, start | (len << 16)));
        bounds_upto(start - kHdr, g0 + k);
      }, hres, (uint32_t)kHold);
    bounds_upto(~0ull, g0 + n);
  }
  if (ABL & 32) {
    asm volatile("s_waitcnt vmcnt(0)" ::: "memory");
    if (lane == 0) lbe[4 * wg + 3] = wall_clock64();
  }
  if (ABL & 16) {
    asm volatile("s_waitcnt vmcnt(0)" ::: "memory");
    const uint64_t tc3 = __builtin_amdgcn_s_memtime();
    if (lane == 0) {
      atomicAdd(reinterpret_cast<unsigned long long*>(&misc[7]), (unsigned long long)(tc1 - tc0));
      atomicAdd(reinterpret_cast<unsigned long long*>(&misc[8]), (unsigned long long)(tc2 - tc1));
      atomicAdd(reinterpret_cast<unsigned long long*>(&misc[9]), (unsigned long long)(tc3 - tc2));
    }
  }
  const uint64_t nwg = (nblocks + 63) / 64;
  if (lane == 63 && !(ABL & 2)) {
    const uint64_t total = excl + tot, total_e = excl_e + tot_e;
    const uint64_t be = wg * 64 + 64 < nblocks ? wg * 64 + 64 : nblocks;
    fbase[be] = (uint32_t)(total < 0xffffffffull ? total : 0xffffffffull);
    rbase[be] = (uint32_t)(total_e < 0xffffffffull ? total_e : 0xffffffffull);
    if (wg == nwg - 1) {
      misc[M_NFRAGS] = total;
      misc[M_NE] = total_e;
    }
  }
}

__device__ __forceinline__ uint32_t xor3(uint32_t a, uint32_t b, uint32_t c) {
  return __builtin_amdgcn_bitop3_b32(a, b, c, 0x96);
}
__device__ __forceinline__ uint32_t apply_fwd(const uint32_t* __restrict__ fwd, uint32_t lane, uint32_t x) {
  const uint8_t* b = reinterpret_cast<const uint8_t*>(fwd);
  const uint32_t lane4 = 4u * lane;
  auto at = [&](int i) -> uint32_t {
    const uint32_t sh = 4 * i >= 8 ? (x >> (4 * i - 8)) : (x << (8 - 4 * i));
    return *reinterpret_cast<const uint32_t*>(b + (((sh & 0xf00u) | lane4) + 4096u * (uint32_t)i));
  };
  const uint32_t r0 = at(0), r1 = at(1), r2 = at(2), r3 = at(3), r4 = at(4), r5 = at(5), r6 = at(6), r7 = at(7);
  return xor3(xor3(r0, r1, r2), xor3(r3, r4, r5), r6) ^ r7;
}
__device__ __forceinline__ uint32_t apply_op(const uint32_t* __restrict__ c, uint32_t x) {
  uint32_t r = 0;
#pragma unroll
  for (int i = 0; i < 8; ++i) r ^= c[i * 16 + ((x >> (4 * i)) & 15u)];
  return r;
}

__device__ __forceinline__ uint4 load16_slow(const uint8_t* __restrict__ seg, uint64_t seg_len, int64_t o) {
  uint64_t lo = 0, hi = 0;
#pragma unroll 1
  for (int i = 0; i < 16; ++i) {
    const int64_t q = o + i;
    const uint64_t byte = (q >= 0 && (uint64_t)q < seg_len) ? seg[q] : 0u;
    if (i < 8) lo |= byte << (8 * i); else hi |= byte << (8 * (i - 8));
  }
  return make_uint4((uint32_t)lo, (uint32_t)(lo >> 32), (uint32_t)hi, (uint32_t)(hi >> 32));
}
__device__ __forceinline__ uint4 load16_safe(const uint8_t* __restrict__ seg, uint64_t seg_len, int64_t o) {
  if (o >= 0 && (uint64_t)o + 16 <= seg_len) return *reinterpret_cast<const uint4*>(seg + o);
  return load16_slow(seg, seg_len, o);
}


template <int N>
__device__ __forceinline__ uint32_t reg_byte(const uint32_t (&h)[N], uint32_t pos) {
  uint32_t t[N];
#pragma unroll
  for (int i = 0; i < N; ++i) t[i] = h[i];
  const uint32_t wi = pos >> 2;
  int n = N;
#pragma unroll
  for (int bit = 0; bit < 6; ++bit) {
    if (n <= 1) break;
    const bool hi = (wi >> bit) & 1u;
#pragma unroll
    for (int i = 0; i < (N + 1) / 2; ++i) {
      if (i < (n + 1) / 2) t[i] = (2 * i + 1 < n) ? (hi ? t[2 * i + 1] : t[2 * i]) : t[2 * i];
    }
    n = (n + 1) / 2;
  }
  return (t[0] >> (8u * (pos & 3u))) & 0xffu;
}

constexpr int kHeadWords = 16;
constexpr int kTailWords = 8;

__device__ __attribute__((noinline)) uint32_t walk_byte(const uint8_t* __restrict__ seg, const Frag* __restrict__ frags,
                                                        uint32_t start_off, uint32_t f_first, uint32_t f_last,
                                                        uint64_t pos) {
  uint64_t beg = 0;
  for (uint32_t cf = f_first;; ++cf) {
    const Frag f = frags[cf];
    if (pos < beg + f.len || cf >= f_last)
      return seg[(uint64_t)start_off + (uint64_t)f.blk * kBlock + f.start + (pos - beg)];
    beg += f.len;
  }
}

struct RegReader {
  uint32_t h[kHeadWords];
  uint32_t t[kTailWords];
  uint32_t nhead;
  uint64_t tstart;
  uint64_t tend;
  const uint8_t* seg;
  const Frag* frags;
  uint32_t start_off;
  uint32_t f_first, f_last;
  __device__ __forceinline__ uint32_t operator()(uint64_t pos) {
    if (pos < nhead) return reg_byte(h, (uint32_t)pos);
    if (pos >= tstart && pos < tend) return reg_byte(t, (uint32_t)(pos - tstart));
    return walk_byte(seg, frags, start_off, f_first, f_last, pos);
  }
};

template <int N>
__device__ __forceinline__ void load_words(const uint8_t* __restrict__ seg, uint64_t seg_len, uint64_t base,
                                           uint32_t (&w)[N]) {
  if (base + 4u * N <= seg_len) {
#pragma unroll
    for (int k = 0; k < N / 4; ++k) {
      uint4 v;
      __builtin_memcpy(&v, seg + base + 16 * k, 16);
      w[4 * k + 0] = v.x; w[4 * k + 1] = v.y; w[4 * k + 2] = v.z; w[4 * k + 3] = v.w;
    }
  } else {
#pragma unroll
    for (int k = 0; k < N / 4; ++k) {
      const uint4 v = load16_safe(seg, seg_len, (int64_t)(base + 16 * k));
      w[4 * k + 0] = v.x; w[4 * k + 1] = v.y; w[4 * k + 2] = v.z; w[4 * k + 3] = v.w;
    }
  }
}

struct EmitArgs {
  const uint8_t* seg;
  uint64_t seg_len;
  bcw_decode_params p;
  const Frag* frags;
  const uint32_t* fbase;
  const uint32_t* rbase;
  const uint2* bsum;
  bcw_record_table tab;
  uint64_t* misc;
  uint32_t kb_flags;
  uint64_t* kb_stamps;
};


struct EmitState {
  uint64_t acc;
  int64_t nzb;
  uint32_t nzk, nzs;
  uint64_t rec;
};
__device__ __forceinline__ uint2 emit_prefetch(const EmitArgs& A, uint64_t b0, uint32_t lane) {
  return b0 > lane ? A.bsum[b0 - 1 - lane] : make_uint2(0xffff0000u, kSumHasE);
}

__device__ __forceinline__ EmitState emit_state(const EmitArgs& A, uint64_t b0, uint32_t lane, uint2 s, uint32_t rec) {
  EmitState st{0, -1, 0, 0, rec};
  uint64_t acc = 0;
  for (uint64_t top = b0; top > 0;) {
    if (top != b0) {
      const uint64_t q = top - 1 - lane;
      s = top > lane ? A.bsum[q] : make_uint2(0xffff0000u, kSumHasE);
    }
    const uint64_t he = __ballot((s.y & kSumHasE) != 0u);
    const uint32_t stop = he ? (uint32_t)__builtin_ctzll(he) : 63u;
    const bool contrib = lane <= stop;
    uint32_t ta = contrib ? (s.x & 0xffffu) : 0u;
#pragma unroll
    for (int d = 32; d >= 1; d >>= 1) ta += (uint32_t)__shfl_xor((int)ta, d, 64);
    acc += (uint32_t)__builtin_amdgcn_readfirstlane(ta);
    const uint64_t nzm = __ballot(contrib && (s.x >> 16) != 0xffffu);
    if (nzm) {
      const uint32_t L = 63u - __builtin_clzll(nzm);
      st.nzb = (int64_t)(top - 1 - L);
      st.nzk = (uint32_t)__builtin_amdgcn_readlane((int)(s.x >> 16), L);
      st.nzs = (uint32_t)__builtin_amdgcn_readlane((int)(s.y & 0xffffu), L);
    }
    if (he) break;
    top = top > 64 ? top - 64 : 0;
  }
  st.acc = acc;
  return st;
}

template <bool NOSTORE = false, bool NOPARSE = false, typename Hook>
__device__ __forceinline__ void emit_chunks(const EmitArgs& A, const EmitState& es, uint64_t f0, uint64_t f1,
                                            uint32_t lane, Hook&& hook) {
  if (f0 >= f1) {
    hook();
    return;
  }
  const Frag* __restrict__ frags = A.frags;
  const uint32_t start_off = A.p.start_off;
  uint64_t acc = es.acc, off = 0;
  uint32_t first = 0;
  if (es.nzb >= 0) {
    off = (uint64_t)start_off + (uint64_t)es.nzb * kBlock + es.nzs;
    first = A.fbase[es.nzb] + es.nzk;
  }
  uint64_t rec = es.rec;
  const bool hint = A.p.mode == BCW_MODE_HINT;
  for (uint64_t c0 = f0; c0 < f1; c0 += 64) {
    const uint64_t g = c0 + lane;
    const bool valid = g < f1;
    const uint4 fr = reinterpret_cast<const uint4*>(frags)[valid ? g : f1 - 1];
    if (c0 == f0) hook();
    Frag f;
    __builtin_memcpy(&f, &fr, sizeof f);
    if (!valid) f = Frag{};
    const uint32_t len = valid ? f.len : 0u;
    const uint64_t D = (uint64_t)start_off + (uint64_t)f.blk * kBlock + f.start;
    const bool isE = valid && (f.type == BCW_RECORD_FULL || f.type == BCW_RECORD_LAST);
    const uint64_t E = __ballot(isE);
    const uint64_t NZ = __ballot(valid && len > 0);
    const uint32_t S = wave_add_scan(len, lane);
    const uint64_t below = (lane == 0) ? 0ull : (~0ull >> (64 - lane));
    const uint64_t pm = E & below;
    const int prev = pm ? 63 - __builtin_clzll(pm) : -1;
    const uint32_t S_prev = __shfl(S, prev < 0 ? 0 : prev, 64);
    const uint64_t between = (uint64_t)(S - len) - (prev < 0 ? 0u : S_prev);
    const uint64_t acc_before = (prev < 0 ? acc : 0ull) + between;
    const uint64_t range = prev < 0 ? below : (below & ~(~0ull >> (63 - prev)));
    const uint64_t nzr = NZ & range;
    const int fnz = nzr ? __builtin_ctzll(nzr) : 0;
    const uint64_t D_fnz = __shfl(D, fnz, 64);
    const uint64_t V = __ballot(valid);
    const int last_valid = V ? 63 - __builtin_clzll(V) : -1;
    const uint32_t S_tot = __shfl(S, last_valid < 0 ? 0 : last_valid, 64);
    const int lastE = E ? 63 - __builtin_clzll(E) : -1;
    uint64_t acc2, off2;
    uint32_t first2;
    {
      const uint32_t S_lastE = __shfl(S, lastE < 0 ? 0 : lastE, 64);
      const uint64_t after = lastE < 0 ? V : (V & ~(~0ull >> (63 - lastE)));
      const uint64_t nza = NZ & after;
      const int fa = nza ? __builtin_ctzll(nza) : 0;
      const uint64_t D_fa = __shfl(D, fa, 64);
      if (lastE >= 0) {
        acc2 = (uint64_t)(S_tot - S_lastE);
        off2 = D_fa;
        first2 = (uint32_t)(c0 + fa);
      } else {
        acc2 = acc + S_tot;
        if (acc > 0 || !nza) { off2 = off; first2 = first; }
        else { off2 = D_fa; first2 = (uint32_t)(c0 + fa); }
      }
    }
    uint64_t foff;
    uint32_t ffrag;
    if (acc_before == 0) { foff = D; ffrag = (uint32_t)g; }
    else if (prev < 0 && acc > 0) { foff = off; ffrag = first; }
    else { foff = D_fnz; ffrag = (uint32_t)(c0 + fnz); }
    const bool full = f.type == BCW_RECORD_FULL;
    const uint32_t src = full ? (uint32_t)g : ffrag;
    const bool src_here = src >= c0 && src < c0 + 64;
    const uint32_t sw0 = (uint32_t)__shfl((int)f.blk, src_here ? (int)(src - c0) : (int)lane, 64);
    const uint32_t sw1 = (uint32_t)__shfl((int)((uint32_t)f.start | ((uint32_t)f.len << 16)),
                                          src_here ? (int)(src - c0) : (int)lane, 64);
    const bool nx_here = src + 1u >= c0 && src + 1u < c0 + 64;
    const uint32_t sx0 = (uint32_t)__shfl((int)f.blk, nx_here ? (int)(src + 1u - c0) : (int)lane, 64);
    const uint32_t sx1 = (uint32_t)__shfl((int)((uint32_t)f.start | ((uint32_t)f.len << 16)),
                                          nx_here ? (int)(src + 1u - c0) : (int)lane, 64);
    if (isE) {
      const uint64_t size = full ? (uint64_t)len : acc_before + len;
      const uint64_t r = rec + __builtin_popcountll(E & below);
      Frag fs = f;
      if (!full) {
        if (src_here) { fs.blk = sw0; fs.start = (uint16_t)sw1; fs.len = (uint16_t)(sw1 >> 16); }
        else fs = frags[src];
      }
      RegReader rd;
      const uint64_t a0 = (uint64_t)start_off + (uint64_t)fs.blk * kBlock + fs.start;
      uint64_t want = size < 64u ? size : 64u;
      if (want > fs.len) want = fs.len;
      rd.nhead = (uint32_t)want;
      load_words(A.seg, A.seg_len, a0, rd.h);
      rd.tstart = rd.tend = ~0ull;
      if (hint) {
        uint64_t nt = size < 32u ? size : 32u;
        if (nt > len) nt = len;
        rd.tstart = size - nt;
        load_words(A.seg, A.seg_len, D + len - nt, rd.t);
      } else if (want < (size < 64u ? size : 64u)) {
        Frag f2;
        if (nx_here) { f2.blk = sx0; f2.start = (uint16_t)sx1; f2.len = (uint16_t)(sx1 >> 16); }
        else f2 = frags[src + 1u];
        load_words(A.seg, A.seg_len, (uint64_t)start_off + (uint64_t)f2.blk * kBlock + f2.start, rd.t);
        uint64_t n2 = f2.len < 32u ? f2.len : 32u;
        if (n2 > size - want) n2 = size - want;
        rd.tstart = want;
        rd.tend = want + n2;
      } else {
#pragma unroll
        for (int k = 0; k < kTailWords; ++k) rd.t[k] = 0;
      }
      rd.seg = A.seg; rd.frags = frags; rd.start_off = start_off;
      rd.f_first = src; rd.f_last = (uint32_t)g;
      uint8_t status, hdr, flags, etag_off;
      uint64_t key_len, val_len, meta_len, expire, aux0, aux1;
      if (NOPARSE) {
        status = 0; hdr = (uint8_t)rd.h[0]; flags = (uint8_t)rd.h[5]; etag_off = 0;
        key_len = rd.h[6] ^ rd.h[9]; val_len = rd.h[7] ^ rd.h[12]; meta_len = rd.h[8] ^ rd.h[15]; expire = rd.h[10];
        aux0 = rd.t[0]; aux1 = rd.t[1];
      } else {
        parse_record(A.p, rd, size, status, hdr, flags, etag_off, key_len, val_len, meta_len, expire, aux0, aux1);
      }
      const bcw_record_table& tab = A.tab;
      if (NOSTORE) {
        if (status == 0xeeu) tab.foff[r] = foff ^ size ^ expire ^ aux0 ^ aux1 ^ key_len ^ val_len ^ meta_len ^ hdr ^ flags ^ etag_off;
      } else if (r < tab.capacity) {
        tab.foff[r] = foff;
        tab.size[r] = size;
        tab.expire[r] = expire;
        if (tab.aux0) tab.aux0[r] = aux0;
        if (tab.aux1) tab.aux1[r] = aux1;
        tab.key_len[r] = (uint32_t)key_len;
        tab.val_len[r] = (uint32_t)val_len;
        tab.meta_len[r] = (uint32_t)meta_len;
        tab.first_frag[r] = src;
        tab.emit_frag[r] = (uint32_t)g;
        tab.hdr_size[r] = hdr;
        tab.flags[r] = flags;
        tab.etag_off[r] = etag_off;
        tab.status[r] = status;
      }
      if (status != BCW_ST_OK) atomicMin((unsigned long long*)&A.misc[M_FIRST_BAD], (unsigned long long)r);
    }
    rec += __builtin_popcountll(E);
    acc = acc2;
    off = off2;
    first = first2;
  }
}

struct ItemMeta {
  uint64_t bb;
  uint2 s;
  uint32_t f0, f1, rec;
};
__device__ __forceinline__ uint32_t ld_const(const uint32_t* p, uint64_t i) {
  return ((const __attribute__((address_space(4))) uint32_t*)p)[i];
}
__device__ __forceinline__ ItemMeta item_meta(const EmitArgs& A, uint64_t it, uint64_t bpw, uint64_t cb0, uint64_t cb1,
                                              uint32_t lane) {
  ItemMeta m;
  m.bb = cb0 + it * bpw < cb1 ? cb0 + it * bpw : cb1 - 1;
  const uint64_t be = m.bb + bpw < cb1 ? m.bb + bpw : cb1;
  m.s = emit_prefetch(A, m.bb, lane);
  m.f0 = ld_const(A.fbase, m.bb);
  m.f1 = ld_const(A.fbase, be);
  m.rec = ld_const(A.rbase, m.bb);
  return m;
}

__device__ __forceinline__ void finalize(const EmitArgs& A, uint64_t nblocks, uint64_t frag_cap, uint32_t tail_panic, uint64_t gen,
                         bcw_decode_result* __restrict__ res, uint32_t lane) {
  uint64_t* misc = A.misc;
  const uint64_t bad_crc = __hip_atomic_load(&misc[M_BAD_CRC], __ATOMIC_RELAXED, __HIP_MEMORY_SCOPE_AGENT);
  const uint64_t bad_type = __hip_atomic_load(&misc[M_BAD_TYPE], __ATOMIC_RELAXED, __HIP_MEMORY_SCOPE_AGENT);
  const uint64_t fb = __hip_atomic_load(&misc[M_FIRST_BAD], __ATOMIC_RELAXED, __HIP_MEMORY_SCOPE_AGENT);
  const uint64_t nfr = __hip_atomic_load(&misc[M_NFRAGS], __ATOMIC_RELAXED, __HIP_MEMORY_SCOPE_AGENT);
  const uint64_t abort_site = __hip_atomic_load(&misc[M_ABORT], __ATOMIC_RELAXED, __HIP_MEMORY_SCOPE_AGENT);
  const uint64_t err = bad_crc < bad_type ? bad_crc : bad_type;
  uint64_t lim = err < frag_cap ? err : frag_cap;
  uint64_t nrec = __hip_atomic_load(&misc[M_NE], __ATOMIC_RELAXED, __HIP_MEMORY_SCOPE_AGENT);
  if (lim < nfr && abort_site == 0ull) {
    uint64_t lo = 0, hi = nblocks;
    while (hi - lo > 1) {
      const uint64_t step = (hi - lo + 63) / 64;
      const uint64_t q = lo + (uint64_t)lane * step;
      const bool le = q < hi && A.fbase[q] <= lim;
      const uint64_t m = __ballot(le);
      const uint32_t L = m ? 63u - __builtin_clzll(m) : 0u;
      lo = lo + (uint64_t)L * step;
      hi = lo + step < hi ? lo + step : hi;
    }
    uint64_t cnt = 0;
    for (uint64_t c0 = A.fbase[lo]; c0 < lim; c0 += 64) {
      const uint64_t g = c0 + lane;
      const uint32_t ty = g < lim ? A.frags[g].type : 0u;
      cnt += (uint64_t)__builtin_popcountll(__ballot(ty == BCW_RECORD_FULL || ty == BCW_RECORD_LAST));
    }
    nrec = (uint64_t)A.rbase[lo] + cnt;
  }
  if (lane != 0) return;
  bcw_decode_result r{};
  r.n_records = nrec;
  r.n_records_total = nrec;
  r.err_frag = err;
  r.err_class = err == ~0ull ? BCW_ERR_NONE : (bad_crc <= bad_type ? BCW_ERR_CRC : BCW_ERR_TYPE);
  r.n_frags = err != ~0ull ? err + 1 : nfr;
  if (r.err_class == BCW_ERR_NONE && tail_panic) r.err_class = BCW_ERR_PANIC;
  if (abort_site != 0ull) {
    r.err_class = BCW_ERR_INTERNAL;
    r.err_frag = abort_site;
    r.n_records = r.n_records_total = 0;
    nrec = 0;
  }
  r.err_file_off = 0;
  if (err != ~0ull && err < frag_cap && abort_site == 0ull) {
    const Frag f = A.frags[err];
    r.err_file_off = (uint64_t)A.p.start_off + (uint64_t)f.blk * kBlock + f.start - kHdr;
  }
  r.first_bad_record = fb < nrec ? (int32_t)(fb < 0x7fffffffull ? fb : 0x7fffffffull) : -1;
  r.n_blocks = nblocks;
  r.retry_frag_capacity = (nfr > frag_cap && abort_site == 0ull) ? nfr : 0;
  r.generation = gen;
  *res = r;
  if (abort_site != 0ull) misc[M_NFRAGS] = 0;
  misc[M_DONE_CRC] = 0;
  misc[M_BAD_CRC] = ~0ull;
  misc[M_FIRST_BAD] = ~0ull;
  misc[M_BAD_TYPE] = ~0ull;
  misc[M_ABORT] = 0;
}

struct StreamFrag {
  int64_t gs, ge;
  uint32_t J;
};

struct SliceLane2 {
  uint32_t base;
  uint32_t sel[4];
};
__device__ __forceinline__ SliceLane2 slice_lane2(uint32_t lane) {
  SliceLane2 s;
  const uint32_t g = (lane >> 3) & 3u, copy = lane & 7u;
  s.base = 0;
#pragma unroll
  for (uint32_t k = 0; k < 4; ++k) {
    const uint32_t slot = (k + g) & 3u;
    s.base |= (slot * 32u + copy * 4u) << (8u * k);
    s.sel[k] = 0x0c0c0000u | ((4u + slot) << 8) | k;
  }
  return s;
}
template <bool SH>
__device__ __forceinline__ uint32_t slice4_step2(const uint8_t* __restrict__ tb, const SliceLane2& sl, uint32_t x,
                                                 uint32_t next) {
  constexpr uint32_t o = SH ? 128u : 0u;
  const uint32_t a0 = *reinterpret_cast<const uint32_t*>(tb + __builtin_amdgcn_perm(x, sl.base, sl.sel[0]) + o);
  const uint32_t a1 = *reinterpret_cast<const uint32_t*>(tb + __builtin_amdgcn_perm(x, sl.base, sl.sel[1]) + o);
  const uint32_t a2 = *reinterpret_cast<const uint32_t*>(tb + __builtin_amdgcn_perm(x, sl.base, sl.sel[2]) + o);
  const uint32_t a3 = *reinterpret_cast<const uint32_t*>(tb + __builtin_amdgcn_perm(x, sl.base, sl.sel[3]) + o);
  return xor3(xor3(a0, a1, a2), a3, next);
}
template <bool CAP>
__device__ __forceinline__ uint32_t chain_piece2(const uint8_t* __restrict__ tb, const SliceLane2& sl, uint32_t seed,
                                                 const uint32_t (&w)[kSPW], uint32_t K = 0, uint32_t* cap = nullptr) {
  uint32_t x = seed ^ w[0];
  uint32_t st[kSPW - 1];
#pragma unroll
  for (int q = 0; q < kSPW - 1; ++q) {
    x = slice4_step2<false>(tb, sl, x, w[q + 1]);
    if (CAP) st[q] = x ^ w[q + 1];
  }
  if (CAP) *cap = K == 1u ? st[0] : (K == 2u ? st[1] : st[2]);
  return slice4_step2<true>(tb, sl, x, 0u);
}

__device__ __forceinline__ uint64_t c_safe_bound(uint64_t seg_len) { return (seg_len + 4u + kSChunk - 1u) / kSChunk; }

__device__ __forceinline__ uint4 lds_entry(const uint32_t* __restrict__ tab, uint32_t idx) {
  return *reinterpret_cast<const uint4*>(tab + 4u * idx);
}
__device__ __forceinline__ void mask_gap(uint32_t (&x)[kSPW], const uint32_t (&w)[kSPW], int32_t pb, uint32_t J,
                                         uint32_t lane, const uint32_t* __restrict__ lds) {
  const uint32_t g = min((uint32_t)(pb - (int32_t)(kSPiece * lane) + 6), (uint32_t)(kS2GapN - 1));
  const uint4 S = lds_entry(lds + kS2Gap, g);
  x[0] = __builtin_amdgcn_perm(J, w[0], S.x);
  x[1] = __builtin_amdgcn_perm(J, w[1], S.y);
  x[2] = __builtin_amdgcn_perm(J, w[2], S.z);
  x[3] = __builtin_amdgcn_perm(J, w[3], S.w);
}
__device__ __forceinline__ void mask_chunk(uint32_t (&x)[kSPW], const uint32_t (&w)[kSPW], int32_t pa, int32_t pb,
                                           int32_t pc, uint32_t J, uint32_t lane, const uint32_t* __restrict__ lds) {
  const int32_t q = (int32_t)(kSPiece * lane);
  const uint4 A = lds_entry(lds + kS2Ge, (uint32_t)min(max(pa - q, 0), kS2GeN - 1));
  const uint4 B = lds_entry(lds + kS2Ge, (uint32_t)min(max(pb - q, 0), kS2GeN - 1));
  const uint4 C = lds_entry(lds + kS2Ge, (uint32_t)min(max(pc - q, 0), kS2GeN - 1));
  const uint4 Js = lds_entry(lds + kS2Jsel, min((uint32_t)(pb - q + 3), (uint32_t)(kS2JselN - 1)));
  auto one = [&](uint32_t wj, uint32_t a, uint32_t b, uint32_t c, uint32_t js) {
    const uint32_t keep = __builtin_amdgcn_bitop3_b32(a, b, c, 0xBA);
    const uint32_t sel = __builtin_amdgcn_bitop3_b32(keep, 0x03020100u, js, 0xCA);
    return __builtin_amdgcn_perm(J, wj, sel);
  };
  x[0] = one(w[0], A.x, B.x, C.x, Js.x);
  x[1] = one(w[1], A.y, B.y, C.y, Js.y);
  x[2] = one(w[2], A.z, B.z, C.z, Js.z);
  x[3] = one(w[3], A.w, B.w, C.w, Js.w);
}
__device__ __forceinline__ uint32_t apply_op_b(const uint32_t* __restrict__ t, uint32_t x) {
  const uint32_t a0 = t[x & 0xffu], a1 = t[256 + ((x >> 8) & 0xffu)];
  const uint32_t a2 = t[512 + ((x >> 16) & 0xffu)], a3 = t[768 + (x >> 24)];
  return xor3(a0, a1, a2) ^ a3;
}

template <bool FASTONLY = false>
__device__ __forceinline__ void stream_verify(const uint8_t* __restrict__ seg, uint64_t seg_len,
                                              uint8_t* __restrict__ fok, const uint4* __restrict__ srec, uint64_t f0,
                                              uint32_t nfr, const uint32_t* __restrict__ lds, uint32_t lane,
                                              uint64_t* __restrict__ misc, uint32_t* __restrict__ s_rem,
                                              uint32_t wslot, const uint8_t* __restrict__ dummy) {
  constexpr int D = 8;
  if (nfr == 0) return;
  const uint8_t* tb = reinterpret_cast<const uint8_t*>(lds + kS2SliceOff);
  const uint32_t* s_lop = lds + kS2LopOff;
  const uint32_t* s_kop = lds + kS2KopOff;
  const SliceLane2 sl = slice_lane2(lane);
  const uint4* rd = srec + f0;
  const uint4 r0 = rd[0], r1 = rd[nfr - 1u];
  const uint32_t cf = r0.y;
  uint64_t c_end = ((uint64_t)r1.x * kSChunk + (r1.w & 1023u) + 4u + kSChunk - 1u) / kSChunk;
  if (c_end > c_safe_bound(seg_len)) c_end = c_safe_bound(seg_len);
  if (c_end < cf || c_end - cf > (1u << 20)) c_end = cf;
  const uint32_t nch = (uint32_t)(c_end - cf);
  struct G32 { int32_t gs, ge; uint32_t J; };
  constexpr int32_t kFar = 0x40000000;
  auto geo = [&](uint4 r) -> G32 {
    return G32{(int32_t)(((r.y - cf) << 10) + ((r.w >> 10) & 1023u)), (int32_t)(((r.x - cf) << 10) + (r.w & 1023u)),
               r.z};
  };
  uint32_t i = 0;
  uint4 rc = r0;
  uint4 rn = rd[1];
  uint32_t ev = 0;
  uint32_t H = 0;
  uint64_t okm = 0;
  uint32_t bad = 0xffffffffu;
  auto flush = [&](uint32_t from, uint32_t n) {
    if (lane < n) fok[f0 + from + lane] = (uint8_t)((okm >> lane) & 1u);
    const uint64_t fail = ~okm & (n == 64u ? ~0ull : (1ull << n) - 1ull);
    if (fail != 0ull && bad == 0xffffffffu) bad = from + (uint32_t)__builtin_ctzll(fail);
  };
  auto close = [&](const uint32_t (&x)[kSPW], uint32_t Lfull, uint32_t K3) {
    uint32_t cap = 0;
    const uint32_t s8 = chain_piece2<true>(tb, sl, H, x, K3, &cap);
    const uint32_t Lsplit = K3 != 0u ? Lfull : 64u;
    const uint32_t K = K3;
    const bool full = lane < Lfull, split = lane == Lsplit;
    const uint32_t A = full ? s8 : apply_op_b(s_kop + (split ? K : 0u) * 1024u, split ? cap : H);
    const uint32_t T = wave_scan_z(apply_fwd(s_lop, lane, A), [](uint32_t a, uint32_t b) { return a ^ b; });
    if (__builtin_amdgcn_readlane(T, 63) == 0u) okm |= 1ull << (i & 63u);
    H = s8 ^ A;
    ++i;
    if ((i & 63u) == 0u) {
      flush(i - 64u, 64u);
      okm = 0;
    }
    rc = rn;
    rn = rd[i + 1u];
  };
  auto close_pb = [&](const uint32_t (&x)[kSPW], int32_t pb) {
    const uint32_t e = (uint32_t)(pb + 4), K = ((e % kSPiece) + 3u) >> 2;
    close(x, e / kSPiece + (K == (uint32_t)kSPW ? 1u : 0u), K & 3u);
  };
  auto slow = [&](uint32_t c, const uint32_t (&w)[kSPW]) {
    const int32_t C0 = (int32_t)(c * kSChunk), C1 = C0 + kSChunk;
    uint32_t nev;
    const bool usual = ((rc.w & kRecUsual) != 0u) & (rc.x - cf == c) & (rn.x - cf > c) & (i + 1u < nfr);
    if (usual) {
      uint32_t x[kSPW];
      mask_gap(x, w, (int32_t)(rc.w & 1023u), rc.z, lane, lds);
      close(x, (rc.w >> 22) & 127u, rc.w >> 29);
      nev = rc.x - cf;
    } else {
      auto rel = [&](int32_t p) -> int32_t { return min(max(p - C0, -64), 4096); };
      G32 fc = i < nfr ? geo(rc) : G32{kFar, kFar, 0u};
      for (;;) {
        if (fc.gs >= C1) break;
        const G32 fn = i + 1u < nfr ? geo(rn) : G32{kFar, kFar, 0u};
        const bool closes = fc.ge + 4 <= C1;
        const bool next_in = closes && fn.gs < C1 && fn.ge >= C1;
        uint32_t x[kSPW];
        const int32_t pa = rel(fc.gs), pb = rel(fc.ge);
        if (next_in && pa <= 0 && fn.gs - fc.ge == (int32_t)kHdr)
          mask_gap(x, w, pb, fc.J, lane, lds);
        else
          mask_chunk(x, w, pa, pb, next_in ? rel(fn.gs) : 4096, fc.J, lane, lds);
        if (!closes) {
          H = chain_piece2<false>(tb, sl, H, x);
          break;
        }
        close_pb(x, pb);
        fc = fn;
        if (next_in) break;
      }
      nev = fc.gs < C1 ? max((uint32_t)fc.ge / (uint32_t)kSChunk, c + 1u) : c + 1u;
    }
    ev = nev;
  };
  auto step = [&](uint32_t c, const uint32_t (&w)[kSPW]) {
    if (FASTONLY || c != ev) H = chain_piece2<false>(tb, sl, H, w);
    else slow(c, w);
  };
  const uint64_t c_safe = seg_len / kSChunk;
  const uint32_t nl = c_safe > cf ? (uint32_t)min(c_safe - cf, (uint64_t)nch) : 0u;
  if (nl > 0u) {
    const uint8_t* wseg = seg + (uint64_t)cf * kSChunk;
    const uint32_t lane16 = lane * kSPiece;
    typedef uint32_t v4u __attribute__((ext_vector_type(4)));
    v4u buf[D];
    auto issue = [&](uint32_t c, v4u& w) {
      const uint8_t* p = c < nl ? wseg + (size_t)c * kSChunk : dummy;
      asm volatile("global_load_dwordx4 %0, %1, %2 nt" : "=v"(w) : "v"(lane16), "s"(p) : "memory");
    };
#pragma unroll
    for (int k = 0; k < D; ++k) issue((uint32_t)k, buf[k]);
    for (uint32_t c = 0; c < nl; c += D) {
      const uint32_t left = nl - c;
      if (lane == 0) s_rem[wslot] = left;
      const uint4 r = *reinterpret_cast<const uint4*>(s_rem + (wslot & ~3u));
      const uint32_t mx = max(max(r.x, r.y), max(r.z, r.w));
      if (left + (uint32_t)D >= mx) __builtin_amdgcn_s_setprio(2);
      else __builtin_amdgcn_s_setprio(0);
#pragma unroll
      for (int k = 0; k < D; ++k) {
        if (c + k < nl) {
          asm volatile("s_waitcnt vmcnt(%1)" : "+v"(buf[k]) : "n"(D - 1));
          const uint32_t w[kSPW] = {buf[k].x, buf[k].y, buf[k].z, buf[k].w};
          step(c + k, w);
        }
        issue(c + k + D, buf[k]);
      }
    }
    asm volatile("s_waitcnt vmcnt(0)" ::"v"(buf[0]), "v"(buf[1]), "v"(buf[2]), "v"(buf[3]), "v"(buf[4]), "v"(buf[5]),
                 "v"(buf[6]), "v"(buf[7]));
    static_assert(D == 8, "the final wait names every ring register");
  }
  for (uint32_t c = nl; c < nch; ++c) {
    uint32_t w[kSPW];
    const uint4 A = load16_safe(seg, seg_len, (int64_t)(((uint64_t)cf + c) * kSChunk) + lane * kSPiece);
    w[0] = A.x; w[1] = A.y; w[2] = A.z; w[3] = A.w;
    step(c, w);
  }
  flush(i & ~63u, i & 63u);
  if (FASTONLY && H == 0x9e3779b9u) misc[7] = H;
  if (lane == 0) {
    if (bad != 0xffffffffu)
      atomicMin(reinterpret_cast<unsigned long long*>(&misc[M_BAD_CRC]), (unsigned long long)(f0 + bad));
    if (!FASTONLY && i < nfr) atomicMax(reinterpret_cast<unsigned long long*>(&misc[M_ABORT]), 20ull);
  }
}

struct CrcTail {
  EmitArgs ea;
  bcw_decode_result* res;
  uint64_t* misc;
  uint64_t nblocks, frag_cap, gen, cb0, cb1;
  uint32_t tail_panic, nwg_total;
};

struct XBalIn {
  uint64_t t, n;
  uint32_t w, on;
};
__device__ __forceinline__ XBalIn xbal_load(const XBal* __restrict__ xb, uint32_t lane) {
  const uint32_t y = lane & 7u;
  XBalIn v;
  v.t = __hip_atomic_load(&xb->t[y], __ATOMIC_RELAXED, __HIP_MEMORY_SCOPE_AGENT);
  v.n = __hip_atomic_load(&xb->n[y], __ATOMIC_RELAXED, __HIP_MEMORY_SCOPE_AGENT);
  v.w = xb->w[y];
  v.on = xb->on;
  return v;
}
__device__ __forceinline__ void xbal_update(XBal* __restrict__ xb, uint32_t lane, const XBalIn& in) {
  const uint32_t y = lane & 7u;
  const uint64_t t = in.t, n = in.n;
  const float Ty = n && t ? (float)t / (float)n : 0.0f;
  const bool all = __ballot(lane < 8u && Ty > 0.0f) == 0xffull && in.on != 0u;
  float sT = lane < 8u ? Ty : 0.0f;
#pragma unroll
  for (int d = 32; d >= 1; d >>= 1) sT += __shfl_xor(sT, d, 64);
  if (lane < 8u) {
    if (all) {
      const float wy = (float)in.w * (1.0f + 0.5f * ((sT / 8.0f) / Ty - 1.0f));
      const float d = fminf(fmaxf(rintf((wy - 65536.0f) / 256.0f), -51.0f), 64.0f);
      xb->w[y] = (uint32_t)(65536 + 256 * (int32_t)d);
    }
    xb->t[y] = 0;
    xb->n[y] = 0;
  }
}

template <int ABL = 0>
__global__ __launch_bounds__(kCrcThreads) void k_crc(const uint8_t* __restrict__ seg, uint64_t seg_len,
                                                     uint32_t start_off, uint64_t nblocks,
                                                     const uint32_t* __restrict__ fbase, uint8_t* __restrict__ fok,
                                                     const uint4* __restrict__ srec,
                                                     uint64_t frag_cap, Tables tabs, EmitArgs ea,
                                                     uint32_t tail_panic, uint64_t gen,
                                                     bcw_decode_result* __restrict__ res,
                                                     uint64_t* __restrict__ misc, uint64_t cb0, uint64_t cb1,
                                                     uint32_t nwg_total, const uint32_t* __restrict__ wstart,
                                                     XBal* __restrict__ xb) {
  __shared__ __attribute__((aligned(16))) uint32_t lds[kS2Image];
  __shared__ CrcTail s_tail;
  __shared__ uint32_t s_wdone;
  __shared__ uint32_t s_eq;
  __shared__ __attribute__((aligned(16))) uint32_t s_rem[kCrcWaves];
  __shared__ uint32_t s_sdone;
  __shared__ unsigned long long s_tsum;
  __shared__ uint64_t s_t0;
  const uint32_t tid = threadIdx.x;
  const uint32_t lane = tid & 63u;
  const uint32_t wave = __builtin_amdgcn_readfirstlane(tid >> 6);
  if (tid < (uint32_t)kCrcWaves) s_rem[tid] = 0;
  if (ea.kb_stamps && lane == 0) {
    uint64_t* q = ea.kb_stamps + 8 * ((uint64_t)blockIdx.x * kCrcWaves + wave);
    q[4] = wall_clock64();
    q[5] = __builtin_amdgcn_s_memtime();
    q[7] = ((uint64_t)__builtin_amdgcn_s_getreg(20 | (31 << 11)) << 32) | __builtin_amdgcn_s_getreg(4 | (31 << 11));
  }
  if (tid == 0) {
    s_wdone = 0;
    s_eq = 0;
    s_sdone = 0;
    s_tsum = 0;
    s_t0 = wall_clock64();
    s_tail = CrcTail{ea, res, misc, nblocks, frag_cap, gen, cb0, cb1, tail_panic, nwg_total};
  }
  {
    const uint4* src4 = reinterpret_cast<const uint4*>(tabs.lds_image2);
    uint4* dst4 = reinterpret_cast<uint4*>(lds);
    constexpr uint32_t kLop4 = kS2SliceOff / 4, kKop4 = kS2KopOff / 4, kEnd4 = kS2Image / 4;
    constexpr uint32_t kN4 = kLop4 + (kEnd4 - kKop4);
    constexpr int kPer = (int)((kN4 + kCrcThreads - 1) / kCrcThreads);
    static_assert(kS2Slice == 256 * 64 && kCrcThreads * 2 == 256 * 8, "slice rows: 256 x 8 distinct dwords");
    auto at = [](uint32_t i) { return i < kLop4 ? i : i - kLop4 + kKop4; };
    uint4 v[kPer];
#pragma unroll
    for (int k2 = 0; k2 < kPer; ++k2) {
      const uint32_t i = tid + k2 * kCrcThreads;
      v[k2] = i < kN4 ? src4[at(i)] : make_uint4(0, 0, 0, 0);
    }
    const uint32_t* src1 = tabs.lds_image2 + kS2SliceOff;
    uint32_t sv[2];
#pragma unroll
    for (int k2 = 0; k2 < 2; ++k2) {
      const uint32_t t = tid + k2 * kCrcThreads;
      sv[k2] = src1[(t >> 3) * 64u + (t & 7u) * 8u];
    }
#pragma unroll
    for (int k2 = 0; k2 < kPer; ++k2) {
      const uint32_t i = tid + k2 * kCrcThreads;
      if (i < kN4) dst4[at(i)] = v[k2];
    }
#pragma unroll
    for (int k2 = 0; k2 < 2; ++k2) {
      const uint32_t t = tid + k2 * kCrcThreads;
      uint4* d = reinterpret_cast<uint4*>(lds + kS2SliceOff + (t >> 3) * 64u + (t & 7u) * 8u);
      d[0] = make_uint4(sv[k2], sv[k2], sv[k2], sv[k2]);
      d[1] = make_uint4(sv[k2], sv[k2], sv[k2], sv[k2]);
    }
  }
  __syncthreads();
  const uint64_t gw = (uint64_t)blockIdx.x * kCrcWaves + wave;
  const uint64_t f0 = wstart[gw];
  uint64_t f1 = wstart[gw + 1];
  if (f1 > frag_cap) f1 = frag_cap;
  if (f0 > f1) f1 = f0;
  const bool aborted = __builtin_amdgcn_readfirstlane(
                           (uint32_t)__hip_atomic_load(&misc[M_ABORT], __ATOMIC_RELAXED, __HIP_MEMORY_SCOPE_AGENT)) != 0u;
  if (aborted) f1 = f0;
  if (blockIdx.x == 0 && tid == 0) misc[M_T_CRC0] = wall_clock64();
  const uint32_t nfr = f1 > f0 ? (uint32_t)(f1 - f0) : 0u;
  uint64_t n_items = 0;
  auto emit_items = [&](uint64_t max_items) {
    asm volatile("" ::: "memory");
    CrcTail T;
    {
      static_assert(sizeof(CrcTail) % 4 == 0, "CrcTail words");
      const uint32_t* src = reinterpret_cast<const uint32_t*>(&s_tail);
      uint32_t* dst = reinterpret_cast<uint32_t*>(&T);
#pragma unroll
      for (int k = 0; k < (int)(sizeof(CrcTail) / 4); ++k) dst[k] = __builtin_amdgcn_readfirstlane(src[k]);
    }
    const EmitArgs& A = T.ea;
    if ((ABL & 8) || (A.kb_flags & 1u) ||
        __builtin_amdgcn_readfirstlane(
            (uint32_t)__hip_atomic_load(&T.misc[M_ABORT], __ATOMIC_RELAXED, __HIP_MEMORY_SCOPE_AGENT)) != 0u)
      return;
    const uint64_t cb0t = T.cb0, cb1t = T.cb1, fcap = T.frag_cap;
    const uint32_t cnt = (uint32_t)(cb1t - cb0t), G = gridDim.x, wg = blockIdx.x;
    const uint64_t fc0 = A.fbase[cb0t], fc1 = A.fbase[cb1t];
    const uint32_t nf_all = (uint32_t)(fc1 > fc0 ? (fc1 - fc0 < fcap ? fc1 - fc0 : fcap) : 0);
    uint32_t bpw = nf_all ? (64u * cnt) / nf_all : cnt;
    if (bpw < 1u) bpw = 1u;
    bpw = __builtin_amdgcn_readfirstlane(bpw);
    const uint32_t cq = cnt / G, cr = cnt % G;
    const uint32_t B0 = cq * wg + (cr * wg) / G, B1 = cq * (wg + 1u) + (cr * (wg + 1u)) / G;
    const uint64_t i0 = __builtin_amdgcn_readfirstlane((B0 + bpw - 1u) / bpw),
                   nitems = __builtin_amdgcn_readfirstlane((B1 + bpw - 1u) / bpw);
    auto deq = [&]() -> uint64_t {
      uint32_t j = 0;
      if (lane == 0) j = atomicAdd(&s_eq, 1u);
      j = __builtin_amdgcn_readfirstlane(j);
      return i0 + j;
    };
    uint64_t taken = 0;
    uint64_t it = deq();
    ItemMeta m = item_meta(A, it, bpw, cb0t, cb1t, lane);
    while (it < nitems) {
      ++taken;
      const EmitState es = emit_state(A, m.bb, lane, m.s, m.rec);
      const uint64_t mf1 = m.f1 < fcap ? m.f1 : fcap;
      uint64_t nx = ~0ull;
      ItemMeta mn = m;
      emit_chunks<(ABL & 4096) != 0, (ABL & 131072) != 0>(A, es, m.f0, mf1, lane, [&]() {
        if (taken < max_items) {
          nx = deq();
          mn = item_meta(A, nx, bpw, cb0t, cb1t, lane);
        }
      });
      it = nx;
      m = mn;
    }
    n_items += taken;
  };
  if (ABL & 64) emit_items(~0ull);
  if (ABL & 16384) {
    for (uint32_t q = 0; q < 4u; ++q) {
      const uint32_t a = nfr * q / 4u, b = nfr * (q + 1u) / 4u;
      stream_verify<(ABL & 8388608) != 0>(seg, seg_len, fok, srec, f0 + a, b - a, lds, lane, misc, s_rem,
                                          (wave & 3u) * 4u + (wave >> 2),
                                          reinterpret_cast<const uint8_t*>(tabs.lds_image2));
    }
  } else if (!(ABL & 32768))
    stream_verify<(ABL & 8388608) != 0>(seg, seg_len, fok, srec, f0, nfr, lds, lane, misc, s_rem,
                                        (wave & 3u) * 4u + (wave >> 2),
                                        reinterpret_cast<const uint8_t*>(tabs.lds_image2));
  __builtin_amdgcn_s_setprio(0);
  if (lane == 0) {
    atomicAdd(&s_tsum, (unsigned long long)(wall_clock64() - s_t0));
    if (atomicAdd(&s_sdone, 1u) == kCrcWaves - 1u) {
      const uint32_t c = blockIdx.x & 7u;
      __hip_atomic_fetch_add(&xb->t[c], (uint64_t)s_tsum, __ATOMIC_RELAXED, __HIP_MEMORY_SCOPE_AGENT);
      __hip_atomic_fetch_add(&xb->n[c], (uint64_t)kCrcWaves, __ATOMIC_RELAXED, __HIP_MEMORY_SCOPE_AGENT);
    }
  }
  if (ea.kb_stamps && lane == 0) {
    uint64_t* q = ea.kb_stamps + 8 * ((uint64_t)blockIdx.x * kCrcWaves + wave);
    q[0] = wall_clock64();
    q[3] = nfr;
  }
  if (!(ABL & 64)) emit_items(~0ull);
  asm volatile("" ::: "memory");
  CrcTail T;
  {
    const uint32_t* src = reinterpret_cast<const uint32_t*>(&s_tail);
    uint32_t* dst = reinterpret_cast<uint32_t*>(&T);
#pragma unroll
    for (int k = 0; k < (int)(sizeof(CrcTail) / 4); ++k) dst[k] = __builtin_amdgcn_readfirstlane(src[k]);
  }
  const EmitArgs& A = T.ea;
  if (A.kb_stamps && lane == 0) {
    uint64_t* q = A.kb_stamps + 8 * ((uint64_t)__builtin_amdgcn_workgroup_id_x() * kCrcWaves + wave);
    q[1] = wall_clock64(); q[2] = n_items;
    q[6] = __builtin_amdgcn_s_memtime();
  }
  asm volatile("s_waitcnt vmcnt(0)" ::: "memory");
  __builtin_amdgcn_fence(__ATOMIC_RELEASE, "workgroup");
  uint32_t order = 0;
  if (lane == 0) order = atomicAdd(&s_wdone, 1u);
  order = __builtin_amdgcn_readlane(order, 0);
  if (order != kCrcWaves - 1) return;
  __builtin_amdgcn_fence(__ATOMIC_ACQUIRE, "workgroup");
  uint64_t gorder = 0;
  if (lane == 0)
    gorder = __hip_atomic_fetch_add(&T.misc[M_DONE_CRC], 1ull, __ATOMIC_RELAXED, __HIP_MEMORY_SCOPE_AGENT);
  gorder = (uint64_t)__shfl((long long)gorder, 0, 64);
  if (gorder != T.nwg_total - 1u) return;
  if (lane == 0) T.misc[M_T_FIN] = wall_clock64();
  const XBalIn xin = xbal_load(xb, lane);
  finalize(A, T.nblocks, T.frag_cap, T.tail_panic, T.gen, T.res, lane);
  xbal_update(xb, lane, xin);
}

__global__ void k_export_frags(const Frag* __restrict__ frags, const uint8_t* __restrict__ fok,
                               const uint64_t* __restrict__ misc, uint64_t cap,
                               uint32_t start_off, bcw_frag_table out, const uint32_t* __restrict__ initc) {
  const uint64_t g = blockIdx.x * (uint64_t)blockDim.x + threadIdx.x;
  const uint64_t n = misc[M_NFRAGS];
  if (g >= n || g >= cap || g >= out.capacity) return;
  const Frag f = frags[g];
  out.data_off[g] = (uint64_t)start_off + (uint64_t)f.blk * kBlock + f.start;
  out.len[g] = f.len;
  const uint32_t u = ~(f.chk ^ initc[f.len]);
  out.stored_crc[g] = ((u >> 15) | (u << 17)) + 0xa282ead8u;
  out.type[g] = f.type;
  out.crc_ok[g] = fok[g];
}



hipError_t launch_decode(const uint8_t* d_seg, const bcw_decode_params& p, const bcw_record_table& t,
                         bcw_decode_result* d_result, const Tables& tabs, Scratch& s, uint64_t nblocks,
                         uint64_t gen, hipStream_t stream, int num_cus, Prof* prof) {
  Prof dummy;
  Prof& pr = prof ? *prof : dummy;
  hipEvent_t ev = nullptr;
  const uint64_t tail = (p.seg_len - p.start_off) % kBlock;
  const uint32_t tail_panic = (tail > 0 && tail < kHdr) ? 1u : 0u;
  const uint32_t nb_grid = (uint32_t)(((nblocks + 63) / 64 + 7) / 8 * 8);
  const EmitArgs ea{d_seg, p.seg_len, p, s.frags, s.fbase, s.rbase, s.bsum, t, s.misc, 0u, nullptr};
  pr.begin(K_CHASE, stream, ev);
  k_chase<0><<<nb_grid, 64, 0, stream>>>(d_seg, p.seg_len, p.start_off, nblocks, s.fbase, s.rbase, s.bsum, s.frags,
                                        s.srec, s.frag_cap, s.lb, s.lbe, s.misc, s.epoch, tabs.initc, s.chase_direct,
                                        s.test_abort_wg, s.wstart, (uint32_t)num_cus * kCrcWaves, s.xbal, s.xbal_on);
  s.test_abort_wg = 0;
  pr.end(K_CHASE, stream, ev);
  if ((++s.epoch & 0xffffffull) == 0) {
    (void)hipMemsetAsync(s.lb, 0, s.nlb * sizeof(uint64_t), stream);
    (void)hipMemsetAsync(s.lbe, 0, s.nlb * sizeof(uint64_t), stream);
    s.epoch = 1;
  }
  pr.begin(K_CRC, stream, ev);
  k_crc<0><<<(uint32_t)num_cus, kCrcThreads, 0, stream>>>(d_seg, p.seg_len, p.start_off, nblocks, s.fbase, s.fok,
                                                         s.srec, s.frag_cap, tabs, ea,
                                                         tail_panic, gen, d_result, s.misc, 0ull, nblocks,
                                                         (uint32_t)num_cus, s.wstart, s.xbal);
  pr.end(K_CRC, stream, ev);
  return hipGetLastError();
}

hipError_t launch_export_frags(const Scratch& s, const bcw_frag_table& out, uint32_t start_off, hipStream_t stream,
                               uint64_t n, const uint32_t* initc) {
  if (n == 0) return hipSuccess;
  k_export_frags<<<(uint32_t)((n + 255) / 256), 256, 0, stream>>>(s.frags, s.fok, s.misc, s.frag_cap, start_off, out,
                                                                    initc);
  return hipGetLastError();
}

}
```

### bitcaskdb_amd/csrc/bcw_internal.h

```cpp
#pragma once
#include <hip/hip_runtime.h>
#include <cstdint>
#include <vector>

#include "bcw.h"

namespace bcw {

constexpr uint32_t kBlock = BCW_BLOCK_SIZE;
constexpr uint32_t kHdr = BCW_HEADER_SIZE;
constexpr uint32_t kWin = 128;
constexpr int kWaveLanes = 64;

struct XBal {
  uint32_t w[8];
  uint32_t pad0[8];
  uint64_t t[8];
  uint64_t n[8];
  uint32_t on;
  uint32_t pad[7];
};
struct Frag {
  uint32_t blk;
  uint16_t start;
  uint16_t len;
  uint32_t chk;
  uint8_t type;
  uint8_t ok;
  uint16_t pad;
};
static_assert(sizeof(Frag) == 16, "Frag layout");

constexpr int kPow2Ops = 16;

struct Tables {
  uint32_t* initc;
  uint32_t* lds_image2;
  uint32_t* enc_ops;
  uint32_t* pow2;
};
constexpr int kOpInv = 40, kOpPow2 = 56, kOpPow2Inv = 88;
constexpr int kEncOpsWords = 103 * 128;

constexpr int kSPiece = 16;
constexpr int kSChunk = 64 * kSPiece;
constexpr int kSPW = kSPiece / 4;
constexpr int kS2Slice = 256 * 64, kS2Lop = 8 * 16 * 64, kS2Kop = kSPW * 4 * 256;
constexpr int kS2LopOff = 0, kS2SliceOff = kS2Lop, kS2KopOff = kS2Lop + kS2Slice;
constexpr int kS2GeN = 17, kS2JselN = 20, kS2GapN = 23;
constexpr int kS2Ge = kS2Slice + kS2Lop + kS2Kop, kS2Jsel = kS2Ge + 4 * kS2GeN, kS2Gap = kS2Jsel + 4 * kS2JselN;
constexpr int kS2Image = kS2Gap + 4 * kS2GapN + 4;
#ifndef BCW_CRC_WAVES
#define BCW_CRC_WAVES 16
#endif
constexpr int kCrcWaves = BCW_CRC_WAVES;
constexpr int kCrcThreads = kCrcWaves * 64;

struct Scratch {
  uint64_t nblocks_cap = 0;
  uint64_t frag_cap = 0;
  uint32_t* fbase = nullptr;
  uint32_t* rbase = nullptr;
  uint2* bsum = nullptr;
  uint64_t* lb = nullptr;
  uint64_t* lbe = nullptr;
  uint64_t nlb = 0;
  uint64_t epoch = 1;
  Frag* frags = nullptr;
  uint4* srec = nullptr;
  uint8_t* fok = nullptr;
  uint32_t* wstart = nullptr;
  XBal* xbal = nullptr;
  uint32_t xbal_on = 1;
  uint64_t* misc = nullptr;
  uint32_t chase_direct = BCW_CHASE_DIRECT_MAX;
  uint64_t test_abort_wg = 0;
};

enum KernelId { K_CHASE = 0, K_CRC, K_RETIRED, K_ENC_PREP, K_ENC_SCAN, K_ENC_EVENTS, K_ENC_WRITE, K_ENC_HINT_LAYOUT,
                K_ENC_EVENTS_HINT, K_NUM };
struct Prof {
  uint32_t mask = 0;
  uint32_t every = 1;
  uint32_t seq[K_NUM] = {};
  bool open[K_NUM] = {};
  struct Mark { int kid; hipEvent_t a, b; };
  std::vector<Mark> marks;
  std::vector<hipEvent_t> pool;
  hipEvent_t get() {
    if (!pool.empty()) { hipEvent_t e = pool.back(); pool.pop_back(); return e; }
    hipEvent_t e = nullptr;
    (void)hipEventCreate(&e);
    return e;
  }
  bool on(int kid) const { return (mask >> kid) & 1u; }
  void begin(int kid, hipStream_t s, hipEvent_t& a) {
    open[kid] = on(kid) && (seq[kid]++ % every) == 0;
    if (open[kid]) { a = get(); (void)hipEventRecord(a, s); }
  }
  void end(int kid, hipStream_t s, hipEvent_t a) {
    if (!open[kid]) return;
    open[kid] = false;
    hipEvent_t b = get();
    (void)hipEventRecord(b, s);
    marks.push_back({kid, a, b});
  }
};

hipError_t launch_decode(const uint8_t* d_seg, const bcw_decode_params& p, const bcw_record_table& t,
                         bcw_decode_result* d_result, const Tables& tabs, Scratch& s, uint64_t nblocks,
                         uint64_t gen, hipStream_t stream, int num_cus, Prof* prof);
hipError_t launch_export_frags(const Scratch& s, const bcw_frag_table& out, uint32_t start_off, hipStream_t stream,
                               uint64_t n, const uint32_t* initc);

struct EncScratch {
  uint64_t rows_cap = 0;
  uint32_t* sz = nullptr;
  uint8_t* mflag = nullptr;
  uint32_t* dsrc = nullptr;
  uint64_t* da = nullptr;
  uint64_t* hda = nullptr;
  uint32_t* hsz = nullptr;
  uint64_t* dpos = nullptr;
  uint64_t* hpos = nullptr;
  void* tiles = nullptr;
  void* ev = nullptr;
  uint32_t* evb = nullptr;
  uint64_t* evt = nullptr;
  uint16_t* hnl = nullptr;
  uint32_t* evw = nullptr;
  void* recdesc = nullptr;
  uint32_t* wl = nullptr;
  uint64_t* emisc = nullptr;
  int wcopy_resident = 0;
  hipStream_t aux = nullptr;
  hipEvent_t ev_scan = nullptr, ev_hscan = nullptr, ev_desc = nullptr;
};

struct EncLaunch {
  const uint8_t* d_src;
  bcw_encode_params p;
  bcw_record_table table;
  uint64_t rows;
  const bcw_decode_result* d_src_result;
  const uint8_t* d_keep;
  bcw_encode_out out;
  bcw_encode_result* d_result;
  const Frag* frags;
  const uint32_t* crc_ops;
  const uint32_t* initc;
  int num_cus;
  uint64_t gen;
};

hipError_t launch_encode(const EncLaunch& L, EncScratch& s, hipStream_t stream, Prof* prof);
size_t enc_sizeof_ev();
size_t enc_sizeof_recdesc();
size_t enc_sizeof_tile();
int enc_tile_items();
int enc_ev_win();

struct DeviceGuard {
  int prev = -1;
  bool ok = false;
  explicit DeviceGuard(int dev) {
    if (hipGetDevice(&prev) != hipSuccess) prev = -1;
    ok = hipSetDevice(dev) == hipSuccess;
  }
  ~DeviceGuard() {
    if (prev >= 0) (void)hipSetDevice(prev);
  }
  DeviceGuard(const DeviceGuard&) = delete;
  DeviceGuard& operator=(const DeviceGuard&) = delete;
};

bcw_ctx* index_ctx(const bcw_index* ix);
constexpr int kIxCounters = 16;
int ix_filter_on(bcw_index* x, bcw_ctx* c, const uint8_t* d_seg, const bcw_decode_params* p,
                 const bcw_record_table* d_table, const bcw_decode_result* d_result, uint64_t src_fid, uint8_t* d_keep,
                 uint64_t* d_cnt, bcw_index_result* d_out);

void build_initc(uint32_t* initc);

int sync_decode(bcw_ctx* c, const uint8_t* h_src, const bcw_decode_params& dp, bcw_decode_result& dres);
int ensure_keep(bcw_ctx* c, uint64_t rows);
bcw_decode_params src_params(const uint8_t* h_src, const bcw_encode_params* p);
int encode_to_host(bcw_ctx* c, const bcw_encode_params* p, const bcw_encode_out* h, bcw_encode_result* h_result,
                   const bcw_decode_result& dres);
int encode_run(bcw_ctx* c, const bcw_encode_params* p, const bcw_encode_out* h, bcw_encode_result* h_result,
               bcw_encode_out* d_out);
int encode_copy_out(bcw_ctx* c, const bcw_encode_params* p, const bcw_encode_out* h, const bcw_encode_result& r,
                    const bcw_encode_out& d, const bcw_decode_result& dres);

struct IxSink {
  virtual ~IxSink() = default;
  virtual int room(uint64_t n, uint64_t key_bytes) = 0;
  uint8_t* keys = nullptr;
  uint64_t* koff = nullptr;
  uint64_t* fid = nullptr;
  uint64_t* off = nullptr;
  uint64_t* size = nullptr;
};
int ix_export(bcw_index* x, const uint64_t* h_fids, uint64_t n_fids, IxSink& sink, uint64_t* n_out,
              uint64_t* key_bytes);

}

struct bcw_ctx {
  int device = 0;
  uint64_t id = 0;
  uint64_t gen_seq = 0;
  uint64_t frag_gen = 0;
  int num_cus = 256;
  hipStream_t own = nullptr;
  hipStream_t cur = nullptr;
  bcw::Tables tabs{};
  bcw::Scratch s{};
  bcw::EncScratch es{};
  uint8_t* d_keep = nullptr;
  uint64_t d_keep_cap = 0;
  void* d_eout = nullptr;
  uint64_t d_eout_cap = 0;
  bcw_encode_result* d_eres = nullptr;
  uint64_t frag_hint = 0;
  uint8_t* d_seg = nullptr;
  uint64_t d_seg_cap = 0;
  void* d_tab_mem = nullptr;
  uint64_t d_tab_cap = 0;
  bcw_record_table d_tab{};
  bcw_decode_result* d_result = nullptr;
  bcw_index_result* d_ires = nullptr;
  uint32_t last_start_off = 0;
  uint32_t chase_direct = BCW_CHASE_DIRECT_MAX;
  uint64_t test_abort_wg = 0;
  bool filter_snapshot = false;
  uint64_t last_nfrag_cap = 0;
  bcw::Prof prof;
};
```

Measured before the change: 4962 GiB/s.

## Compute CRC wave boundaries in k_crc via ballot search, drop wstart table

The chase kernel no longer writes a per-wave start-fragment table (wstart) while emitting fragments. Each CRC wave now finds its own fragment range at kernel start with a ballot-driven search over fragment start offsets inside the owning block, overlapped with the LDS table setup. The chase kernel is also launched with four waves per workgroup, with the extra waves presumably taking over part of the emit work. This removes the serial boundary loop and global writes from chase but adds search latency and extra fragment loads to the start of every CRC wave.

```diff
diff --git a/bitcaskdb_amd/csrc/bcw_api.cpp b/bitcaskdb_amd/csrc/bcw_api.cpp
--- a/bitcaskdb_amd/csrc/bcw_api.cpp
+++ b/bitcaskdb_amd/csrc/bcw_api.cpp
@@ -322,7 +322,6 @@
   (void)hipFree(s.frags);
   (void)hipFree(s.srec);
   (void)hipFree(s.fok);
-  (void)hipFree(s.wstart);
   (void)hipFree(s.xbal);
   (void)hipFree(s.misc);
   s = Scratch{};
@@ -396,7 +395,6 @@
             hipMalloc(&s.lbe, nwg * 8) == hipSuccess && hipMalloc(&s.frags, fc * sizeof(Frag)) == hipSuccess &&
             hipMalloc(&s.srec, (fc + 4) * sizeof(uint4)) == hipSuccess &&
             hipMalloc(&s.fok, fc) == hipSuccess &&
-            hipMalloc(&s.wstart, ((size_t)c->num_cus * kCrcWaves + 1) * 4) == hipSuccess &&
             hipMalloc(&s.xbal, sizeof(XBal)) == hipSuccess &&
             hipMalloc(&s.misc, 16 * sizeof(uint64_t)) == hipSuccess;
   if (!ok) { free_scratch(s); return BCW_E_NOMEM; }
diff --git a/bitcaskdb_amd/csrc/bcw_decode.hip b/bitcaskdb_amd/csrc/bcw_decode.hip
--- a/bitcaskdb_amd/csrc/bcw_decode.hip
+++ b/bitcaskdb_amd/csrc/bcw_decode.hip
@@ -172,14 +172,13 @@
 struct WavePart {
   ClassW cw;
   uint64_t L, nwaves, round16, den16, C;
-  double rden, rC;
+  double rden;
   __device__ __forceinline__ WavePart(const ClassW& c, uint64_t L_, uint64_t nwaves_) : cw(c), L(L_), nwaves(nwaves_) {
     const uint32_t G = (uint32_t)(nwaves / kCrcWaves);
     round16 = 16ull * cw.p8;
     den16 = round16 * (G / 8u) + 16ull * cw.prefix(G % 8u);
     C = L / 1024u;
     rden = 1.0 / (double)den16;
-    rC = C ? 1.0 / (double)C : 0.0;
   }
   __device__ __forceinline__ uint64_t P(uint64_t v) const {
     if (v >= nwaves) return L;
@@ -188,19 +187,6 @@
     const uint64_t num16 = round16 * (r / 8u) + 16ull * cw.prefix(y) + cw.weight(y) * (v % kCrcWaves);
     return 1024u * div_floor(num16 * C, den16, rden);
   }
-  __device__ __forceinline__ uint64_t first_at(uint64_t x) const {
-    if (C == 0) return x == 0 ? 0 : nwaves;
-    const uint64_t X = (x + 1023u) / 1024u, N = div_floor(X * den16 + C - 1, C, rC);
-    const uint32_t q = (uint32_t)N / (uint32_t)round16;
-    const uint64_t rem = N - (uint64_t)q * round16;
-    uint32_t y = 0;
-#pragma unroll
-    for (uint32_t k = 1; k < 8; ++k) y += 16ull * cw.prefix(k) <= rem ? 1u : 0u;
-    const uint64_t wy = cw.weight(y), base = 16ull * cw.prefix(y);
-    const uint32_t jj = (uint32_t)(rem - base + wy - 1) / (uint32_t)wy;
-    const uint64_t v = ((uint64_t)q * 8u + y) * kCrcWaves + jj;
-    return v < nwaves ? v : nwaves;
-  }
 };
 
 __device__ __forceinline__ ClassW class_weights(uint32_t xw) {
@@ -218,24 +204,25 @@
   return c;
 }
 
+constexpr int kChaseWaves = 4;
 template <int ABL = 0>
-__global__ __launch_bounds__(64) void k_chase(const uint8_t* __restrict__ seg, uint64_t seg_len, uint32_t start_off,
-                                              uint64_t nblocks, uint32_t* __restrict__ fbase,
-                                              uint32_t* __restrict__ rbase, uint2* __restrict__ bsum,
-                                              Frag* __restrict__ frags, uint4* __restrict__ srec, uint64_t frag_cap,
-                                              uint64_t* __restrict__ lb,
-                                              uint64_t* __restrict__ lbe, uint64_t* __restrict__ misc,
-                                              uint64_t epoch, const uint32_t* __restrict__ initc,
-                                              uint32_t direct_max, uint64_t test_abort_wg,
-                                              uint32_t* __restrict__ wstart, uint32_t nwaves,
-                                              XBal* __restrict__ xb, uint32_t xb_on) {
+__global__ __launch_bounds__(64 * kChaseWaves) void k_chase(const uint8_t* __restrict__ seg, uint64_t seg_len,
+                                                            uint32_t start_off, uint64_t nblocks,
+                                                            uint32_t* __restrict__ fbase, uint32_t* __restrict__ rbase,
+                                                            uint2* __restrict__ bsum, Frag* __restrict__ frags,
+                                                            uint4* __restrict__ srec, uint64_t frag_cap,
+                                                            uint64_t* __restrict__ lb, uint64_t* __restrict__ lbe,
+                                                            uint64_t* __restrict__ misc, uint64_t epoch,
+                                                            const uint32_t* __restrict__ initc, uint32_t direct_max,
+                                                            uint64_t test_abort_wg) {
   constexpr int kHold = (ABL & 256) ? 16 : kChaseHold;
   __shared__ uint32_t s_hold[kHold][2][64];
   __shared__ uint8_t s_type[kHold][64];
-  const uint32_t lane = threadIdx.x;
-  const uint32_t xw = lane < 8u ? (xb_on ? xb->w[lane] : 65536u) : 0u;
-  const uint64_t tc0 = (ABL & 16) ? __builtin_amdgcn_s_memtime() : 0;
-  if ((ABL & 32) && threadIdx.x == 0) lbe[4 * blockIdx.x] = wall_clock64();
+  __shared__ uint64_t s_g0[64];
+  __shared__ uint32_t s_n[64];
+  __shared__ uint32_t s_hres[64];
+  const uint32_t lane = threadIdx.x & 63u;
+  const uint32_t wv = __builtin_amdgcn_readfirstlane(threadIdx.x >> 6);
   const uint64_t wg = blockIdx.x;
   if (wg >= (nblocks + 63) / 64) return;
   const uint64_t b = wg * 64 + lane;
@@ -245,202 +232,200 @@
     boff = (uint64_t)start_off + b * kBlock;
     bufsize = (uint32_t)((seg_len - boff) < kBlock ? (seg_len - boff) : kBlock);
   }
-  uint32_t ne = 0, tacc = 0, tnz = 0xffffu, tst = 0, badk = 0xffffffffu;
-  uint32_t hres = 0;
-  const uint32_t n = chase_block(seg, seg_len, boff, bufsize,
-                                 [&](uint32_t k, uint32_t start, uint32_t len, uint32_t crc, uint32_t type) {
-                                   if (k < (uint32_t)kHold) {
-                                     s_hold[k][0][lane] = crc;
-                                     s_hold[k][1][lane] = start | (len << 16);
-                                     s_type[k][lane] = (uint8_t)type;
-                                   }
-                                   if (k == (uint32_t)kHold - 1u) hres = start + len;
-                                   if (type == BCW_RECORD_FULL || type == BCW_RECORD_LAST) {
-                                     ++ne;
-                                     tacc = 0;
-                                     tnz = 0xffffu;
-                                   } else {
-                                     if (len > 0 && tnz == 0xffffu) { tnz = k; tst = start; }
-                                     tacc += len;
-                                     if ((type < BCW_RECORD_FULL || type > BCW_RECORD_LAST) && badk == 0xffffffffu) badk = k;
-                                   }
-                                 });
-  const uint64_t tc1 = (ABL & 16) ? __builtin_amdgcn_s_memtime() : 0;
-  if ((ABL & 32) && lane == 0) lbe[4 * wg + 1] = wall_clock64();
-  if (wg == 0 && lane == 0) xb->on = xb_on;
-  const uint32_t incl = wave_add_scan(n, lane);
-  const uint32_t tot = __builtin_amdgcn_readlane(incl, 63);
-  const uint32_t incl_e = wave_add_scan(ne, lane);
-  const uint32_t tot_e = __builtin_amdgcn_readlane(incl_e, 63);
-  const uint64_t tag = epoch << 40;
-  const uint64_t nwg_all = (nblocks + 63) / 64;
-  const bool force = wg + 1 == test_abort_wg;
-  uint64_t excl = 0, excl_e = 0;
-  const uint32_t nh = n < (uint32_t)kHold ? n : (uint32_t)kHold;
-  auto held_checks = [&]() {
-    if (ABL & 2) return;
-    constexpr uint32_t kWb = 16;
-    static_assert(kHold % kWb == 0, "held-header batches stay inside s_hold");
-    for (uint32_t k0 = 0; k0 < nh; k0 += kWb) {
-      uint32_t ic[kWb];
-#pragma unroll
-      for (uint32_t q = 0; q < kWb; ++q) ic[q] = initc[k0 + q < nh ? s_hold[k0 + q][1][lane] >> 16 : 0u];
-#pragma unroll
-      for (uint32_t q = 0; q < kWb; ++q)
-        if (k0 + q < nh) s_hold[k0 + q][0][lane] = check_word(s_hold[k0 + q][0][lane], ic[q]);
-    }
-  };
-  if (ABL & 1) {
-    held_checks();
-  } else if (nwg_all <= (uint64_t)direct_max) {
-    if (lane == 0)
-      __hip_atomic_store(&lb[wg], tag | (kLbAgg << 38) | tot | ((uint64_t)tot_e << 19), __ATOMIC_RELAXED,
-                         __HIP_MEMORY_SCOPE_AGENT);
-    uint64_t v[kDirect / 64];
-#pragma unroll
-    for (int k = 0; k < kDirect / 64; ++k) {
-      const uint64_t q = lane + 64u * k;
-      v[k] = q < wg ? __hip_atomic_load(&lb[q], __ATOMIC_RELAXED, __HIP_MEMORY_SCOPE_AGENT) : tag;
-    }
-    held_checks();
-    Spin sp;
-    if (force) sp.lim = 0;
-    for (;;) {
-      bool wait = force;
-#pragma unroll
-      for (int k = 0; k < kDirect / 64; ++k) wait |= (v[k] >> 40) != epoch;
-      if (!__builtin_amdgcn_readfirstlane((uint32_t)(__ballot(wait) != 0ull))) break;
-      if (!sp.go(misc, 9)) {
-#pragma unroll
-        for (int k = 0; k < kDirect / 64; ++k)
-          if ((v[k] >> 40) != epoch) v[k] = 0;
-        break;
-      }
+  const bool next_hdr = b + 1 < nblocks && seg_len - (boff + kBlock) >= kHdr;
+  uint64_t tc0 = 0, tc1 = 0, tc2 = 0;
+  if (wv == 0) {
+    tc0 = (ABL & 16) ? __builtin_amdgcn_s_memtime() : 0;
+    if ((ABL & 32) && lane == 0) lbe[4 * blockIdx.x] = wall_clock64();
+    uint32_t ne = 0, tacc = 0, tnz = 0xffffu, tst = 0, badk = 0xffffffffu;
+    uint32_t hres = 0;
+    const uint32_t n = chase_block(seg, seg_len, boff, bufsize,
+                                   [&](uint32_t k, uint32_t start, uint32_t len, uint32_t crc, uint32_t type) {
+                                     if (k < (uint32_t)kHold) {
+                                       s_hold[k][0][lane] = crc;
+                                       s_hold[k][1][lane] = start | (len << 16);
+                                       s_type[k][lane] = (uint8_t)type;
+                                     }
+                                     if (k == (uint32_t)kHold - 1u) hres = start + len;
+                                     if (type == BCW_RECORD_FULL || type == BCW_RECORD_LAST) {
+                                       ++ne;
+                                       tacc = 0;
+                                       tnz = 0xffffu;
+                                     } else {
+                                       if (len > 0 && tnz == 0xffffu) { tnz = k; tst = start; }
+                                       tacc += len;
+                                       if ((type < BCW_RECORD_FULL || type > BCW_RECORD_LAST) && badk == 0xffffffffu) badk = k;
+                                     }
+                                   });
+    tc1 = (ABL & 16) ? __builtin_amdgcn_s_memtime() : 0;
+    if ((ABL & 32) && lane == 0) lbe[4 * wg + 1] = wall_clock64();
+    const uint32_t incl = wave_add_scan(n, lane);
+    const uint32_t tot = __builtin_amdgcn_readlane(incl, 63);
+    const uint32_t incl_e = wave_add_scan(ne, lane);
+    const uint32_t tot_e = __builtin_amdgcn_readlane(incl_e, 63);
+    const uint64_t tag = epoch << 40;
+    const uint64_t nwg_all = (nblocks + 63) / 64;
+    const bool force = wg + 1 == test_abort_wg;
+    uint64_t excl = 0, excl_e = 0;
+    const uint32_t nh = n < (uint32_t)kHold ? n : (uint32_t)kHold;
+    auto held_checks = [&]() {
+      if (ABL & 2) return;
+      constexpr uint32_t kWb = 16;
+      static_assert(kHold % kWb == 0, "held-header batches stay inside s_hold");
+      for (uint32_t k0 = 0; k0 < nh; k0 += kWb) {
+        uint32_t ic[kWb];
+#pragma unroll
+        for (uint32_t q = 0; q < kWb; ++q) ic[q] = initc[k0 + q < nh ? s_hold[k0 + q][1][lane] >> 16 : 0u];
+#pragma unroll
+        for (uint32_t q = 0; q < kWb; ++q)
+          if (k0 + q < nh) s_hold[k0 + q][0][lane] = check_word(s_hold[k0 + q][0][lane], ic[q]);
+      }
+    };
+    if (ABL & 1) {
+      held_checks();
+    } else if (nwg_all <= (uint64_t)direct_max) {
+      if (lane == 0)
+        __hip_atomic_store(&lb[wg], tag | (kLbAgg << 38) | tot | ((uint64_t)tot_e << 19), __ATOMIC_RELAXED,
+                           __HIP_MEMORY_SCOPE_AGENT);
+      uint64_t v[kDirect / 64];
 #pragma unroll
       for (int k = 0; k < kDirect / 64; ++k) {
         const uint64_t q = lane + 64u * k;
-        if ((v[k] >> 40) != epoch) v[k] = __hip_atomic_load(&lb[q], __ATOMIC_RELAXED, __HIP_MEMORY_SCOPE_AGENT);
-      }
-    }
-    uint64_t c = 0, ce = 0;
-#pragma unroll
-    for (int k = 0; k < kDirect / 64; ++k) {
-      const uint64_t q = lane + 64u * k;
-      if (q < wg) {
-        c += v[k] & 0x7ffffu;
-        ce += (v[k] >> 19) & 0x7ffffu;
-      }
-    }
-#pragma unroll
-    for (int d = 32; d >= 1; d >>= 1) {
-      c += (uint64_t)__shfl_xor((long long)c, d, 64);
-      ce += (uint64_t)__shfl_xor((long long)ce, d, 64);
-    }
-    excl = c;
-    excl_e = ce;
-  } else {
-    const uint64_t fl = (wg == 0 ? kLbInc : kLbAgg) << 38;
-    if (lane == 0) {
-      __hip_atomic_store(&lb[wg], tag | fl | tot, __ATOMIC_RELAXED, __HIP_MEMORY_SCOPE_AGENT);
-      __hip_atomic_store(&lbe[wg], tag | fl | tot_e, __ATOMIC_RELAXED, __HIP_MEMORY_SCOPE_AGENT);
-    }
-    held_checks();
-    bool dn = false, de = false;
-    for (uint64_t top = wg; top > 0 && !(dn && de);) {
-      const uint64_t q = top - 1 - lane;
-      uint64_t vn = 0, ve = 0;
-      if (top > lane) {
-        Spin sp;
-        if (force) sp.lim = 0;
-        if (!dn)
-          while (((vn = __hip_atomic_load(&lb[q], __ATOMIC_RELAXED, __HIP_MEMORY_SCOPE_AGENT)) >> 40) != epoch || force)
-            if (!sp.go(misc, 10)) { vn = 0; break; }
-        if (!de)
-          while (((ve = __hip_atomic_load(&lbe[q], __ATOMIC_RELAXED, __HIP_MEMORY_SCOPE_AGENT)) >> 40) != epoch || force)
-            if (!sp.go(misc, 11)) { ve = 0; break; }
-      }
-      auto step = [&](uint64_t v, bool& done, uint64_t& acc) {
-        if (done) return;
-        const uint64_t inc = __ballot(top > lane && ((v >> 38) & 3u) == kLbInc);
-        const uint32_t stop = inc ? (uint32_t)__builtin_ctzll(inc) : 64u;
-        uint64_t c = (lane <= stop && top > lane) ? (v & kLbMask) : 0ull;
-#pragma unroll
-        for (int d = 32; d >= 1; d >>= 1) c += (uint64_t)__shfl_xor((long long)c, d, 64);
-        acc += c;
-        done = inc != 0;
-      };
-      step(vn, dn, excl);
-      step(ve, de, excl_e);
-      top = top > 64 ? top - 64 : 0;
-    }
-    if (lane == 0 && wg != 0) {
-      __hip_atomic_store(&lb[wg], tag | (kLbInc << 38) | ((excl + tot) & kLbMask), __ATOMIC_RELAXED,
-                         __HIP_MEMORY_SCOPE_AGENT);
-      __hip_atomic_store(&lbe[wg], tag | (kLbInc << 38) | ((excl_e + tot_e) & kLbMask), __ATOMIC_RELAXED,
-                         __HIP_MEMORY_SCOPE_AGENT);
-    }
-  }
-  const uint64_t g0 = excl + incl - n;
-  const uint64_t tc2 = (ABL & 16) ? __builtin_amdgcn_s_memtime() : 0;
-  if ((ABL & 32) && lane == 0) lbe[4 * wg + 2] = wall_clock64();
-  if (b < nblocks && !(ABL & 2)) {
-    fbase[b] = (uint32_t)(g0 < 0xffffffffull ? g0 : 0xffffffffull);
-    const uint64_t r0 = excl_e + incl_e - ne;
-    rbase[b] = (uint32_t)(r0 < 0xffffffffull ? r0 : 0xffffffffull);
-    bsum[b] = make_uint2(tacc | (tnz << 16), tst | (ne ? kSumHasE : 0u));
-    if (badk != 0xffffffffu)
-      atomicMin(reinterpret_cast<unsigned long long*>(&misc[M_BAD_TYPE]), (unsigned long long)(g0 + badk));
-    const bool next_hdr = b + 1 < nblocks && seg_len - (boff + kBlock) >= kHdr;
-    auto adj = [&](uint32_t k, uint32_t sl_k) { return k + 1u < n || (next_hdr && (sl_k & 0xffffu) + (sl_k >> 16) == kBlock); };
-    const uint64_t L = seg_len - start_off, rel = boff - start_off;
-    const WavePart wp(class_weights(xw), L, nwaves);
-    const uint64_t span = b + 1 == nblocks ? ~0ull : (uint64_t)kBlock - 1;
-    uint64_t w = wp.first_at(rel);
-    uint64_t bw = wp.P(w) - rel;
-    auto bounds_upto = [&](uint64_t hp, uint64_t idx) __attribute__((always_inline)) {
-      const uint64_t h = hp < span ? hp : span;
-      while (w <= nwaves && bw <= h) {
-        wstart[w] = (uint32_t)(idx < 0xffffffffull ? idx : 0xffffffffull);
-        ++w;
-        bw = wp.P(w) - rel;
-      }
-    };
-    for (uint32_t k = 0; k < nh; ++k) {
-      const uint32_t sl = s_hold[k][1][lane];
-      put_frag_J(frags, srec, g0 + k, frag_cap, (uint32_t)b, boff, sl, s_hold[k][0][lane], s_type[k][lane],
-                 adj(k, sl));
-      bounds_upto((sl & 0xffffu) - kHdr, g0 + k);
-    }
-    if (n > (uint32_t)kHold)
+        v[k] = q < wg ? __hip_atomic_load(&lb[q], __ATOMIC_RELAXED, __HIP_MEMORY_SCOPE_AGENT) : tag;
+      }
+      held_checks();
+      Spin sp;
+      if (force) sp.lim = 0;
+      for (;;) {
+        bool wait = force;
+#pragma unroll
+        for (int k = 0; k < kDirect / 64; ++k) wait |= (v[k] >> 40) != epoch;
+        if (!__builtin_amdgcn_readfirstlane((uint32_t)(__ballot(wait) != 0ull))) break;
+        if (!sp.go(misc, 9)) {
+#pragma unroll
+          for (int k = 0; k < kDirect / 64; ++k)
+            if ((v[k] >> 40) != epoch) v[k] = 0;
+          break;
+        }
+#pragma unroll
+        for (int k = 0; k < kDirect / 64; ++k) {
+          const uint64_t q = lane + 64u * k;
+          if ((v[k] >> 40) != epoch) v[k] = __hip_atomic_load(&lb[q], __ATOMIC_RELAXED, __HIP_MEMORY_SCOPE_AGENT);
+        }
+      }
+      uint64_t c = 0, ce = 0;
+#pragma unroll
+      for (int k = 0; k < kDirect / 64; ++k) {
+        const uint64_t q = lane + 64u * k;
+        if (q < wg) {
+          c += v[k] & 0x7ffffu;
+          ce += (v[k] >> 19) & 0x7ffffu;
+        }
+      }
+#pragma unroll
+      for (int d = 32; d >= 1; d >>= 1) {
+        c += (uint64_t)__shfl_xor((long long)c, d, 64);
+        ce += (uint64_t)__shfl_xor((long long)ce, d, 64);
+      }
+      excl = c;
+      excl_e = ce;
+    } else {
+      const uint64_t fl = (wg == 0 ? kLbInc : kLbAgg) << 38;
+      if (lane == 0) {
+        __hip_atomic_store(&lb[wg], tag | fl | tot, __ATOMIC_RELAXED, __HIP_MEMORY_SCOPE_AGENT);
+        __hip_atomic_store(&lbe[wg], tag | fl | tot_e, __ATOMIC_RELAXED, __HIP_MEMORY_SCOPE_AGENT);
+      }
+      held_checks();
+      bool dn = false, de = false;
+      for (uint64_t top = wg; top > 0 && !(dn && de);) {
+        const uint64_t q = top - 1 - lane;
+        uint64_t vn = 0, ve = 0;
+        if (top > lane) {
+          Spin sp;
+          if (force) sp.lim = 0;
+          if (!dn)
+            while (((vn = __hip_atomic_load(&lb[q], __ATOMIC_RELAXED, __HIP_MEMORY_SCOPE_AGENT)) >> 40) != epoch || force)
+              if (!sp.go(misc, 10)) { vn = 0; break; }
+          if (!de)
+            while (((ve = __hip_atomic_load(&lbe[q], __ATOMIC_RELAXED, __HIP_MEMORY_SCOPE_AGENT)) >> 40) != epoch || force)
+              if (!sp.go(misc, 11)) { ve = 0; break; }
+        }
+        auto step = [&](uint64_t v, bool& done, uint64_t& acc) {
+          if (done) return;
+          const uint64_t inc = __ballot(top > lane && ((v >> 38) & 3u) == kLbInc);
+          const uint32_t stop = inc ? (uint32_t)__builtin_ctzll(inc) : 64u;
+          uint64_t c = (lane <= stop && top > lane) ? (v & kLbMask) : 0ull;
+#pragma unroll
+          for (int d = 32; d >= 1; d >>= 1) c += (uint64_t)__shfl_xor((long long)c, d, 64);
+          acc += c;
+          done = inc != 0;
+        };
+        step(vn, dn, excl);
+        step(ve, de, excl_e);
+        top = top > 64 ? top - 64 : 0;
+      }
+      if (lane == 0 && wg != 0) {
+        __hip_atomic_store(&lb[wg], tag | (kLbInc << 38) | ((excl + tot) & kLbMask), __ATOMIC_RELAXED,
+                           __HIP_MEMORY_SCOPE_AGENT);
+        __hip_atomic_store(&lbe[wg], tag | (kLbInc << 38) | ((excl_e + tot_e) & kLbMask), __ATOMIC_RELAXED,
+                           __HIP_MEMORY_SCOPE_AGENT);
+      }
+    }
+    const uint64_t g0 = excl + incl - n;
+    tc2 = (ABL & 16) ? __builtin_amdgcn_s_memtime() : 0;
+    if ((ABL & 32) && lane == 0) lbe[4 * wg + 2] = wall_clock64();
+    s_g0[lane] = g0;
+    s_n[lane] = n | (next_hdr ? 0x80000000u : 0u);
+    s_hres[lane] = hres;
+    if (b < nblocks && !(ABL & 2)) {
+      fbase[b] = (uint32_t)(g0 < 0xffffffffull ? g0 : 0xffffffffull);
+      const uint64_t r0 = excl_e + incl_e - ne;
+      rbase[b] = (uint32_t)(r0 < 0xffffffffull ? r0 : 0xffffffffull);
+      bsum[b] = make_uint2(tacc | (tnz << 16), tst | (ne ? kSumHasE : 0u));
+      if (badk != 0xffffffffu)
+        atomicMin(reinterpret_cast<unsigned long long*>(&misc[M_BAD_TYPE]), (unsigned long long)(g0 + badk));
+    }
+    if (lane == 63 && !(ABL & 2)) {
+      const uint64_t total = excl + tot, total_e = excl_e + tot_e;
+      const uint64_t be = wg * 64 + 64 < nblocks ? wg * 64 + 64 : nblocks;
+      fbase[be] = (uint32_t)(total < 0xffffffffull ? total : 0xffffffffull);
+      rbase[be] = (uint32_t)(total_e < 0xffffffffull ? total_e : 0xffffffffull);
+      if (wg == nwg_all - 1) {
+        misc[M_NFRAGS] = total;
+        misc[M_NE] = total_e;
+      }
+    }
+  }
+  __syncthreads();
+  if (!(ABL & 2)) {
+    const uint32_t nw = s_n[lane], n = nw & 0x7fffffffu;
+    const bool nxt = (nw >> 31) != 0u;
+    const uint64_t g0 = s_g0[lane];
+    const uint32_t nh = n < (uint32_t)kHold ? n : (uint32_t)kHold;
+    auto adj = [&](uint32_t k, uint32_t sl_k) { return k + 1u < n || (nxt && (sl_k & 0xffffu) + (sl_k >> 16) == kBlock); };
+    if (b < nblocks)
+      for (uint32_t k = wv; k < nh; k += (uint32_t)kChaseWaves) {
+        const uint32_t sl = s_hold[k][1][lane];
+        put_frag_J(frags, srec, g0 + k, frag_cap, (uint32_t)b, boff, sl, s_hold[k][0][lane], s_type[k][lane],
+                   adj(k, sl));
+      }
+    const uint64_t over = __ballot(b < nblocks && n > (uint32_t)kHold);
+    const uint32_t rank = (uint32_t)__builtin_popcountll(over & ((1ull << lane) - 1ull));
+    if (((over >> lane) & 1ull) && rank % (uint32_t)kChaseWaves == wv)
       chase_block(seg, seg_len, boff, bufsize, [&](uint32_t k, uint32_t start, uint32_t len, uint32_t crc, uint32_t type) {
         put_frag(frags, srec, g0 + k, frag_cap, (uint32_t)b, boff, start, len, crc, type, initc,
                  adj(k, start | (len << 16)));
-        bounds_upto(start - kHdr, g0 + k);
-      }, hres, (uint32_t)kHold);
-    bounds_upto(~0ull, g0 + n);
-  }
-  if (ABL & 32) {
+      }, s_hres[lane], (uint32_t)kHold);
+  }
+  if (ABL & (16 | 32)) {
     asm volatile("s_waitcnt vmcnt(0)" ::: "memory");
-    if (lane == 0) lbe[4 * wg + 3] = wall_clock64();
-  }
-  if (ABL & 16) {
-    asm volatile("s_waitcnt vmcnt(0)" ::: "memory");
-    const uint64_t tc3 = __builtin_amdgcn_s_memtime();
-    if (lane == 0) {
+    __syncthreads();
+    if ((ABL & 32) && threadIdx.x == 0) lbe[4 * wg + 3] = wall_clock64();
+    if ((ABL & 16) && threadIdx.x == 0) {
+      const uint64_t tc3 = __builtin_amdgcn_s_memtime();
       atomicAdd(reinterpret_cast<unsigned long long*>(&misc[7]), (unsigned long long)(tc1 - tc0));
       atomicAdd(reinterpret_cast<unsigned long long*>(&misc[8]), (unsigned long long)(tc2 - tc1));
       atomicAdd(reinterpret_cast<unsigned long long*>(&misc[9]), (unsigned long long)(tc3 - tc2));
-    }
-  }
-  const uint64_t nwg = (nblocks + 63) / 64;
-  if (lane == 63 && !(ABL & 2)) {
-    const uint64_t total = excl + tot, total_e = excl_e + tot_e;
-    const uint64_t be = wg * 64 + 64 < nblocks ? wg * 64 + 64 : nblocks;
-    fbase[be] = (uint32_t)(total < 0xffffffffull ? total : 0xffffffffull);
-    rbase[be] = (uint32_t)(total_e < 0xffffffffull ? total_e : 0xffffffffull);
-    if (wg == nwg - 1) {
-      misc[M_NFRAGS] = total;
-      misc[M_NE] = total_e;
     }
   }
 }
@@ -1072,20 +1057,20 @@
   bcw_decode_result* res;
   uint64_t* misc;
   uint64_t nblocks, frag_cap, gen, cb0, cb1;
-  uint32_t tail_panic, nwg_total;
+  uint32_t tail_panic, nwg_total, xb_on, pad;
 };
 
 struct XBalIn {
   uint64_t t, n;
   uint32_t w, on;
 };
-__device__ __forceinline__ XBalIn xbal_load(const XBal* __restrict__ xb, uint32_t lane) {
+__device__ __forceinline__ XBalIn xbal_load(const XBal* __restrict__ xb, uint32_t lane, uint32_t on) {
   const uint32_t y = lane & 7u;
   XBalIn v;
   v.t = __hip_atomic_load(&xb->t[y], __ATOMIC_RELAXED, __HIP_MEMORY_SCOPE_AGENT);
   v.n = __hip_atomic_load(&xb->n[y], __ATOMIC_RELAXED, __HIP_MEMORY_SCOPE_AGENT);
   v.w = xb->w[y];
-  v.on = xb->on;
+  v.on = on;
   return v;
 }
 __device__ __forceinline__ void xbal_update(XBal* __restrict__ xb, uint32_t lane, const XBalIn& in) {
@@ -1105,6 +1090,59 @@
     xb->t[y] = 0;
     xb->n[y] = 0;
   }
+}
+
+struct Boundary {
+  uint32_t fb0, n;
+  uint32_t t;
+  uint32_t step, sl0, sl1;
+};
+__device__ __forceinline__ uint32_t frag_start_ld(const Frag* __restrict__ frags, uint64_t g) {
+  return reinterpret_cast<const uint32_t*>(frags + g)[1] & 0xffffu;
+}
+__device__ __forceinline__ Boundary boundary_begin(const WavePart& wp, uint64_t v, uint64_t nblocks,
+                                                   const uint32_t* __restrict__ fbase) {
+  Boundary q{0, 0, 0, 0, 0, 0};
+  if (nblocks == 0) return q;
+  const uint64_t P = wp.P(v), bq = P / kBlock;
+  const uint64_t b = bq < nblocks - 1 ? bq : nblocks - 1;
+  const uint64_t r = P - b * kBlock;
+  q.t = (uint32_t)(r < 0x10000ull ? r : 0x10000ull) + kHdr;
+  const uint32_t f0 = ld_const(fbase, b), f1 = ld_const(fbase, b + 1);
+  q.fb0 = f0;
+  q.n = f1 > f0 ? f1 - f0 : 0u;
+  return q;
+}
+__device__ __forceinline__ void boundary_load(const Boundary& q, const Frag* __restrict__ frags, uint64_t frag_cap,
+                                              uint32_t lane, uint32_t lo, uint32_t step, uint32_t& sl0, uint32_t& sl1) {
+  const uint64_t g0 = (uint64_t)q.fb0 + lo + (uint64_t)lane * step, g1 = g0 + 64ull * step;
+  sl0 = frag_start_ld(frags, g0 < frag_cap ? g0 : 0);
+  sl1 = frag_start_ld(frags, g1 < frag_cap ? g1 : 0);
+}
+__device__ __forceinline__ void boundary_probe(Boundary& q, const Frag* __restrict__ frags, uint64_t frag_cap,
+                                               uint32_t lane) {
+  if (q.n == 0u) return;
+  q.step = (q.n + 127u) / 128u;
+  boundary_load(q, frags, frag_cap, lane, 0u, q.step, q.sl0, q.sl1);
+}
+__device__ __forceinline__ uint64_t boundary_end(const Boundary& q, const Frag* __restrict__ frags, uint64_t frag_cap,
+                                                 uint32_t lane) {
+  uint32_t lo = 0, hi = q.n, step = q.step, sl0 = q.sl0, sl1 = q.sl1;
+  while (lo < hi) {
+    const uint32_t i0 = lo + lane * step, i1 = i0 + 64u * step;
+    const uint64_t m0 = __ballot(i0 < hi && (uint64_t)q.fb0 + i0 < frag_cap && sl0 < q.t);
+    const uint64_t m1 = __ballot(i1 < hi && (uint64_t)q.fb0 + i1 < frag_cap && sl1 < q.t);
+    const uint32_t k = (uint32_t)(__builtin_popcountll(m0) + __builtin_popcountll(m1));
+    if (k == 0u) break;
+    const uint32_t h2 = lo + k * step;
+    hi = h2 < hi ? h2 : hi;
+    lo = lo + (k - 1u) * step + 1u;
+    if (lo >= hi) break;
+    step = (hi - lo + 127u) / 128u;
+    boundary_load(q, frags, frag_cap, lane, lo, step, sl0, sl1);
+  }
+  const uint64_t f = (uint64_t)q.fb0 + lo;
+  return f < frag_cap ? f : frag_cap;
 }
 
 template <int ABL = 0>
@@ -1116,8 +1154,7 @@
                                                      uint32_t tail_panic, uint64_t gen,
                                                      bcw_decode_result* __restrict__ res,
                                                      uint64_t* __restrict__ misc, uint64_t cb0, uint64_t cb1,
-                                                     uint32_t nwg_total, const uint32_t* __restrict__ wstart,
-                                                     XBal* __restrict__ xb) {
+                                                     uint32_t nwg_total, XBal* __restrict__ xb, uint32_t xb_on) {
   __shared__ __attribute__((aligned(16))) uint32_t lds[kS2Image];
   __shared__ CrcTail s_tail;
   __shared__ uint32_t s_wdone;
@@ -1126,6 +1163,7 @@
   __shared__ uint32_t s_sdone;
   __shared__ unsigned long long s_tsum;
   __shared__ uint64_t s_t0;
+  __shared__ uint32_t s_bound[kCrcWaves + 1];
   const uint32_t tid = threadIdx.x;
   const uint32_t lane = tid & 63u;
   const uint32_t wave = __builtin_amdgcn_readfirstlane(tid >> 6);
@@ -1142,8 +1180,13 @@
     s_sdone = 0;
     s_tsum = 0;
     s_t0 = wall_clock64();
-    s_tail = CrcTail{ea, res, misc, nblocks, frag_cap, gen, cb0, cb1, tail_panic, nwg_total};
-  }
+    s_tail = CrcTail{ea, res, misc, nblocks, frag_cap, gen, cb0, cb1, tail_panic, nwg_total, xb_on};
+  }
+  const uint64_t gw = (uint64_t)blockIdx.x * kCrcWaves + wave;
+  const bool wlast = wave == (uint32_t)kCrcWaves - 1u;
+  const uint32_t xw = lane < 8u ? (xb_on ? xb->w[lane] : 65536u) : 0u;
+  const uint64_t abort_w = __hip_atomic_load(&misc[M_ABORT], __ATOMIC_RELAXED, __HIP_MEMORY_SCOPE_AGENT);
+  Boundary bq0{0, 0, 0, 0, 0, 0}, bq1{0, 0, 0, 0, 0, 0};
   {
     const uint4* src4 = reinterpret_cast<const uint4*>(tabs.lds_image2);
     uint4* dst4 = reinterpret_cast<uint4*>(lds);
@@ -1165,6 +1208,12 @@
       const uint32_t t = tid + k2 * kCrcThreads;
       sv[k2] = src1[(t >> 3) * 64u + (t & 7u) * 8u];
     }
+    const WavePart wp(class_weights(xw), seg_len > start_off ? seg_len - start_off : 0ull,
+                      (uint64_t)gridDim.x * kCrcWaves);
+    bq0 = boundary_begin(wp, gw, nblocks, fbase);
+    if (wlast) bq1 = boundary_begin(wp, gw + 1, nblocks, fbase);
+    boundary_probe(bq0, ea.frags, frag_cap, lane);
+    if (wlast) boundary_probe(bq1, ea.frags, frag_cap, lane);
 #pragma unroll
     for (int k2 = 0; k2 < kPer; ++k2) {
       const uint32_t i = tid + k2 * kCrcThreads;
@@ -1178,14 +1227,20 @@
       d[1] = make_uint4(sv[k2], sv[k2], sv[k2], sv[k2]);
     }
   }
+  {
+    const uint32_t fa = (uint32_t)boundary_end(bq0, ea.frags, frag_cap, lane);
+    if (lane == 0) s_bound[wave] = fa;
+    if (wlast) {
+      const uint32_t fe = (uint32_t)boundary_end(bq1, ea.frags, frag_cap, lane);
+      if (lane == 0) s_bound[kCrcWaves] = fe;
+    }
+  }
   __syncthreads();
-  const uint64_t gw = (uint64_t)blockIdx.x * kCrcWaves + wave;
-  const uint64_t f0 = wstart[gw];
-  uint64_t f1 = wstart[gw + 1];
+  const uint64_t f0 = __builtin_amdgcn_readfirstlane(s_bound[wave]);
+  uint64_t f1 = __builtin_amdgcn_readfirstlane(s_bound[wave + 1u]);
   if (f1 > frag_cap) f1 = frag_cap;
   if (f0 > f1) f1 = f0;
-  const bool aborted = __builtin_amdgcn_readfirstlane(
-                           (uint32_t)__hip_atomic_load(&misc[M_ABORT], __ATOMIC_RELAXED, __HIP_MEMORY_SCOPE_AGENT)) != 0u;
+  const bool aborted = __builtin_amdgcn_readfirstlane((uint32_t)abort_w) != 0u;
   if (aborted) f1 = f0;
   if (blockIdx.x == 0 && tid == 0) misc[M_T_CRC0] = wall_clock64();
   const uint32_t nfr = f1 > f0 ? (uint32_t)(f1 - f0) : 0u;
@@ -1296,7 +1351,7 @@
   gorder = (uint64_t)__shfl((long long)gorder, 0, 64);
   if (gorder != T.nwg_total - 1u) return;
   if (lane == 0) T.misc[M_T_FIN] = wall_clock64();
-  const XBalIn xin = xbal_load(xb, lane);
+  const XBalIn xin = xbal_load(xb, lane, T.xb_on);
   finalize(A, T.nblocks, T.frag_cap, T.tail_panic, T.gen, T.res, lane);
   xbal_update(xb, lane, xin);
 }
@@ -1329,9 +1384,9 @@
   const uint32_t nb_grid = (uint32_t)(((nblocks + 63) / 64 + 7) / 8 * 8);
   const EmitArgs ea{d_seg, p.seg_len, p, s.frags, s.fbase, s.rbase, s.bsum, t, s.misc, 0u, nullptr};
   pr.begin(K_CHASE, stream, ev);
-  k_chase<0><<<nb_grid, 64, 0, stream>>>(d_seg, p.seg_len, p.start_off, nblocks, s.fbase, s.rbase, s.bsum, s.frags,
-                                        s.srec, s.frag_cap, s.lb, s.lbe, s.misc, s.epoch, tabs.initc, s.chase_direct,
-                                        s.test_abort_wg, s.wstart, (uint32_t)num_cus * kCrcWaves, s.xbal, s.xbal_on);
+  k_chase<0><<<nb_grid, 64 * kChaseWaves, 0, stream>>>(d_seg, p.seg_len, p.start_off, nblocks, s.fbase, s.rbase, s.bsum,
+                                                         s.frags, s.srec, s.frag_cap, s.lb, s.lbe, s.misc, s.epoch,
+                                                         tabs.initc, s.chase_direct, s.test_abort_wg);
   s.test_abort_wg = 0;
   pr.end(K_CHASE, stream, ev);
   if ((++s.epoch & 0xffffffull) == 0) {
@@ -1343,7 +1398,7 @@
   k_crc<0><<<(uint32_t)num_cus, kCrcThreads, 0, stream>>>(d_seg, p.seg_len, p.start_off, nblocks, s.fbase, s.fok,
                                                          s.srec, s.frag_cap, tabs, ea,
                                                          tail_panic, gen, d_result, s.misc, 0ull, nblocks,
-                                                         (uint32_t)num_cus, s.wstart, s.xbal);
+                                                         (uint32_t)num_cus, s.xbal, s.xbal_on);
   pr.end(K_CRC, stream, ev);
   return hipGetLastError();
 }
diff --git a/bitcaskdb_amd/csrc/bcw_internal.h b/bitcaskdb_amd/csrc/bcw_internal.h
--- a/bitcaskdb_amd/csrc/bcw_internal.h
+++ b/bitcaskdb_amd/csrc/bcw_internal.h
@@ -17,8 +17,7 @@
   uint32_t pad0[8];
   uint64_t t[8];
   uint64_t n[8];
-  uint32_t on;
-  uint32_t pad[7];
+  uint32_t pad[8];
 };
 struct Frag {
   uint32_t blk;
@@ -69,7 +68,6 @@
   Frag* frags = nullptr;
   uint4* srec = nullptr;
   uint8_t* fok = nullptr;
-  uint32_t* wstart = nullptr;
   XBal* xbal = nullptr;
   uint32_t xbal_on = 1;
   uint64_t* misc = nullptr;
```

New measurement: 4996 GiB/s, median of 6. About the same (+0.7%).
